# zkemail/zk-email-verify

Hardware: NVIDIA H100
Metric: EmailVerifier proofs/sec (witness+prove) (higher is better)
Workload: dtype u256 (BN254 Fr/Fq integers, 8x32-bit limbs)

## Files before the change

### zk-email-verify_b200/csrc/engine.cu

```cuda
#include "ff.cuh"
namespace zke { namespace dev { unsigned long long g_kernel_launches = 0; } }
#include "witness.cu"
#include "matvec.cu"
#include "ntt.cu"
#include "msm.cuh"
#include "fixed_base.cuh"
namespace zke { namespace dev {
ZKE_DEFINE_CONSTANT_UPLOAD(upload_constants_engine)
cudaError_t upload_constants_msm_g1(const FieldConsts*, const FieldConsts*);
cudaError_t upload_constants_msm_g2(const FieldConsts*, const FieldConsts*);
cudaError_t upload_constants_fixed_base(const FieldConsts*, const FieldConsts*);
cudaError_t upload_constants_verify(const FieldConsts*, const FieldConsts*);
} }

#include "../../include/zkemail_b200.h"
#include "cuda_host.hpp"
#include "engine.hpp"
#include "witness_program.hpp"
#include "binfile.hpp"
#include "ec_host.hpp"
#include "setup_host.hpp"
#include <algorithm>
#include <cstdio>
#include <cstring>
#include <atomic>
#include <memory>
#include <mutex>
#include <thread>
#include <unordered_map>

using namespace zke;

void zke::select_device(int device) {
    int n = 0;
    if (cudaGetDeviceCount(&n) != cudaSuccess || n == 0) throw std::runtime_error("no CUDA device available (this library has no CPU fallback)");
    if (device < 0 || device >= n) throw std::runtime_error("bad device index");
    CUDA_OK(cudaSetDevice(device));
    dev::FieldConsts fr, fq;
    fill_consts(fr, fr_params());
    fill_consts(fq, fq_params());
    CUDA_OK(dev::upload_constants_engine(&fr, &fq));
    CUDA_OK(dev::upload_constants_msm_g1(&fr, &fq));
    CUDA_OK(dev::upload_constants_msm_g2(&fr, &fq));
    CUDA_OK(dev::upload_constants_fixed_base(&fr, &fq));
    CUDA_OK(dev::upload_constants_verify(&fr, &fq));
    CUDA_OK(dev::configure_witness_kernel());
}

namespace {

template <class F>
std::vector<AffineH<F>> window_table(const AffineH<F>& gen) {
    std::vector<AffineH<F>> t(32 * 256, AffineH<F>::inf());
    JacobianH<F> base = JacobianH<F>::from_affine(gen);
    for (int w = 0; w < 32; ++w) {
        JacobianH<F> acc = JacobianH<F>::inf();
        for (int d = 1; d < 256; ++d) {
            acc = acc.add(base);
            t[w * 256 + d] = acc.to_affine();
        }
        for (int k = 0; k < 8; ++k) base = base.dbl();
    }
    return t;
}

std::vector<U256> to_standard(const std::vector<Fr>& v) {
    std::vector<U256> out(v.size());
    const unsigned T = std::max(1u, std::min(16u, std::thread::hardware_concurrency()));
    std::vector<std::thread> th;
    for (unsigned t = 0; t < T; ++t)
        th.emplace_back([&, t]() { for (size_t i = v.size() * t / T; i < v.size() * (t + 1) / T; ++i) out[i] = v[i].to_u256(); });
    for (auto& x : th) x.join();
    return out;
}

}

struct zke_zkey {
    uint32_t n_vars = 0, n_public = 0, log_n = 0;
    int device = 0;
    bool toy = false;
    bool delta_one = false;
    G1AffineH alpha1, beta1, delta1;
    G2AffineH beta2, gamma2, delta2;
    std::vector<G1AffineH> ic;
    DevBuf A, B1, B2, C, H;
    int h_levels = 1;
    dev::MsmConfig cfg_h;
    bool has_coefs = false;
    std::vector<uint32_t> a_ptr, a_var, a_coef, b_ptr, b_var, b_coef;
    std::vector<U256> coefs;
};

struct zke_ctx {
    const zke_circuit* circuit = nullptr;
    const zke_zkey* zkey = nullptr;
    int device = 0;
    uint32_t max_batch = 0;
    uint32_t n_vars = 0, n_public = 0, n_inputs = 0;
    cudaStream_t stream = nullptr;
    DevBuf ops, iter_hdr, lc_terms, aux, coop, coef_r, small_inv;
    std::vector<uint32_t> coef_word;
    std::vector<uint32_t> iter_info;
    DevBuf a_ptr, a_terms, b_ptr, b_terms, c_ptr, c_terms;
    dev::DevProgram prog;
    dev::DevR1cs r1cs;
    DevBuf tw_fwd, tw_inv, coset_scale;
    dev::NttTables ntt;
    size_t stride = 0;
    DevBuf inputs, check_flag;
    uint32_t inputs_resident = 0;
    struct Slot {
        bool allocated = false, busy = false;
        DevBuf w_all, inputs, results, first_bad;
        uint8_t* results_host = nullptr;
        uint8_t* publics_host = nullptr;
        std::vector<cudaEvent_t> done;
        cudaEvent_t witness_done = nullptr;
        uint32_t loaded = 0;
        uint32_t batch = 0;
        std::vector<uint8_t> rs;
    };
    Slot slots[2];
    uint64_t n_submitted = 0, n_collected = 0;
    int shard_rank = -1, shard_world = 0, shard_log_g = 0, shard_stage = 0;
    struct Lane { cudaStream_t st = nullptr, heavy = nullptr; cudaEvent_t ev[6] = {}; DevBuf va, vb, vc, vd, msm_ws; };
    Lane lanes[ZKE_MAX_LANES];
    int n_lanes = 1, lanes_alloc = 0;
    int finish_threads = 4;
    dev::MsmConfig cfg_w, cfg_h;
    bool split_streams = true;
    std::vector<uint32_t> bad_host;
    bool profile = false;
    std::vector<cudaEvent_t> ev_pool;
    size_t ev_used = 0;
    struct Span { int stage; size_t e0, e1; };
    std::vector<Span> spans;
    double stage_ms[ZKE_N_STAGES] = {0};
    uint64_t stage_count[ZKE_N_STAGES] = {0};
    cudaEvent_t ev(size_t* idx) {
        if (ev_used == ev_pool.size()) { cudaEvent_t e; cudaEventCreate(&e); ev_pool.push_back(e); }
        *idx = ev_used;
        return ev_pool[ev_used++];
    }
    size_t mark(cudaStream_t st) { size_t i; cudaEventRecord(ev(&i), st); return i; }
    size_t mark() { return mark(stream); }
    void collect() {
        for (auto& s : spans) {
            float ms = 0;
            if (cudaEventElapsedTime(&ms, ev_pool[s.e0], ev_pool[s.e1]) == cudaSuccess) { stage_ms[s.stage] += ms; stage_count[s.stage]++; }
        }
        spans.clear();
        ev_used = 0;
    }
};

static const uint32_t SETUP_SLAB = 1u << 20;
static void h_table_config(zke_zkey* zk, size_t N) {
    const char* e = getenv("ZKE_H_PRECOMP");
    const bool precomp = !(e && atoi(e) == 0);
    zk->cfg_h = dev::msm_config_full((uint32_t)N, precomp);
    zk->h_levels = precomp ? dev::msm_windows(zk->cfg_h) : 1;
}
static void build_h_levels(zke_zkey* zk, size_t N, uint8_t* scratch, cudaStream_t st) {
    for (int lvl = 1; lvl < zk->h_levels; ++lvl) {
        const uint8_t* prev = zk->H.p + (size_t)(lvl - 1) * N * sizeof(dev::G1Affine);
        uint8_t* cur = zk->H.p + (size_t)lvl * N * sizeof(dev::G1Affine);
        for (size_t off = 0; off < N; off += SETUP_SLAB) {
            uint32_t cnt = (uint32_t)std::min<size_t>(SETUP_SLAB, N - off);
            dev::scale_pow2_batch<dev::Fq>(prev + sizeof(dev::G1Affine) * off, cnt, zk->cfg_h.c, scratch, cur + sizeof(dev::G1Affine) * off, st);
        }
    }
    CHECK_LAUNCH();
    CUDA_OK(cudaStreamSynchronize(st));
}

static zke_zkey* do_setup(const zke_circuit* zc, uint64_t seed, int device) {
    select_device(device);
    const Circuit& c = zc->c;
    SetupScalars S = compute_setup_scalars(c, seed);
    std::unique_ptr<zke_zkey> zk(new zke_zkey());
    zk->n_vars = c.n_vars; zk->n_public = c.n_public(); zk->log_n = S.log_n; zk->device = device;
    zk->toy = true;
    const size_t N = (size_t)1 << S.log_n;
    const uint32_t m = c.n_vars, l = c.n_public();

    G1JacH g1 = G1JacH::from_affine(g1_generator());
    G2JacH g2 = G2JacH::from_affine(g2_generator());
    zk->alpha1 = g1.mul(S.alpha.to_u256()).to_affine();
    zk->beta1 = g1.mul(S.beta.to_u256()).to_affine();
    zk->delta1 = g1.mul(S.delta.to_u256()).to_affine();
    zk->beta2 = g2.mul(S.beta.to_u256()).to_affine();
    zk->gamma2 = g2.mul(S.gamma.to_u256()).to_affine();
    zk->delta2 = g2.mul(S.delta.to_u256()).to_affine();

    DevBuf t1, t2, scal, scratch;
    t1.upload(window_table<Fq>(g1_generator()));
    t2.upload(window_table<Fq2>(g2_generator()));
    const uint32_t SLAB = SETUP_SLAB;
    scratch.alloc((size_t)SLAB * sizeof(dev::G2XYZZ));
    cudaStream_t st = nullptr;

    auto run_g1 = [&](const std::vector<Fr>& s, DevBuf& out) {
        std::vector<U256> std_s = to_standard(s);
        scal.upload(std_s);
        out.alloc(s.size() * sizeof(dev::G1Affine));
        for (size_t off = 0; off < s.size(); off += SLAB) {
            uint32_t cnt = (uint32_t)std::min<size_t>(SLAB, s.size() - off);
            dev::fixed_base_batch<dev::Fq>(t1.p, scal.p + 32 * off, cnt, scratch.p, out.p + sizeof(dev::G1Affine) * off, st);
        }
        CHECK_LAUNCH();
        CUDA_OK(cudaStreamSynchronize(st));
    };
    run_g1(S.a, zk->A);
    run_g1(S.b, zk->B1);
    run_g1(S.kc, zk->C);
    {
        h_table_config(zk.get(), N);
        std::vector<U256> std_s = to_standard(S.h);
        scal.upload(std_s);
        zk->H.alloc((size_t)zk->h_levels * N * sizeof(dev::G1Affine));
        for (size_t off = 0; off < N; off += SLAB) {
            uint32_t cnt = (uint32_t)std::min<size_t>(SLAB, N - off);
            dev::fixed_base_batch<dev::Fq>(t1.p, scal.p + 32 * off, cnt, scratch.p, zk->H.p + sizeof(dev::G1Affine) * off, st);
        }
        build_h_levels(zk.get(), N, scratch.p, st);
    }
    {
        std::vector<U256> std_s = to_standard(S.b);
        scal.upload(std_s);
        zk->B2.alloc((size_t)m * sizeof(dev::G2Affine));
        for (size_t off = 0; off < m; off += SLAB) {
            uint32_t cnt = (uint32_t)std::min<size_t>(SLAB, m - off);
            dev::fixed_base_batch<dev::Fq2>(t2.p, scal.p + 32 * off, cnt, scratch.p, zk->B2.p + sizeof(dev::G2Affine) * off, st);
        }
        CHECK_LAUNCH();
        CUDA_OK(cudaStreamSynchronize(st));
    }
    zk->ic.resize(l + 1);
    CUDA_OK(cudaMemcpy(zk->ic.data(), zk->C.p, sizeof(G1AffineH) * (l + 1), cudaMemcpyDeviceToHost));
    CUDA_OK(cudaMemset(zk->C.p, 0, sizeof(G1AffineH) * (l + 1)));
    return zk.release();
}

namespace {
void split_container(const uint8_t* b, size_t len, SecView sec[11]) {
    if (!b || len < 12 || memcmp(b, "zkey", 4) != 0) throw std::runtime_error("not a .zkey file (bad magic)");
    if (rd32(b + 4) != 1) throw std::runtime_error("unsupported .zkey version");
    for (const BinSection& s : binfile_sections(b, len, ".zkey"))
        if (s.type >= 1 && s.type <= 10) sec[s.type] = s.view;
}

template <class Launch>
int64_t first_flagged(uint32_t* flag, Launch launch) {
    CUDA_OK(cudaMemset(flag, 0xff, 4));
    launch(flag);
    ZKE_COUNT_LAUNCH(1);
    CHECK_LAUNCH();
    uint32_t first = 0;
    CUDA_OK(cudaMemcpy(&first, flag, 4, cudaMemcpyDeviceToHost));
    return first == 0xffffffffu ? -1 : (int64_t)first;
}

template <class F>
__global__ void validate_points_kernel(const uint8_t* __restrict__ pts, uint32_t n, F b, uint32_t* bad) {
    const uint32_t i = blockIdx.x * blockDim.x + threadIdx.x;
    if (i >= n) return;
    const dev::Affine<F> p = dev::Affine<F>::load(pts + sizeof(dev::Affine<F>) * (size_t)i);
    if (p.is_inf()) return;
    if (!dev::below_modulus(p.x) || !dev::below_modulus(p.y) || !(p.y.sqr() == p.x.sqr() * p.x + b)) atomicMin(bad, i);
}

template <class F, class HostF>
int64_t first_invalid_point(const uint8_t* pts, size_t n, const HostF& b_host, uint32_t* flag) {
    if (!n) return -1;
    F b;
    static_assert(sizeof(F) == sizeof(HostF), "host / device field images differ");
    memcpy(&b, &b_host, sizeof(F));
    return first_flagged(flag, [&](uint32_t* f) { validate_points_kernel<F><<<(unsigned)((n + 127) / 128), 128>>>(pts, (uint32_t)n, b, f); });
}

Fq2 g2_twist_b() { return Fq2{Fq::from_u64(3), Fq::zero()} * Fq2{Fq::from_u64(9), Fq::one()}.inv(); }

struct U256HashE {
    size_t operator()(const U256& x) const { return (size_t)(x.v[0] * 0x9E3779B97F4A7C15ull ^ x.v[1] * 31 ^ x.v[2] * 131 ^ x.v[3]); }
};
}

static zke_zkey* do_zkey_load(const SecView sec[11], int device) {
    select_device(device);
    for (int s = 1; s <= 9; ++s) if (!sec[s].p) throw std::runtime_error(".zkey section " + std::to_string(s) + " is missing");
    if (sec[1].n < 4 || rd32(sec[1].p) != 1) throw std::runtime_error("not a Groth16 .zkey (protocol id)");
    const uint8_t* h = sec[2].p;
    const size_t HDR = 4 + 32 + 4 + 32 + 12 + 64 + 64 + 128 + 128 + 64 + 128;
    if (sec[2].n < HDR) throw std::runtime_error(".zkey header section too short");
    if (rd32(h) != 32 || memcmp(h + 4, fq_params().p.v, 32) != 0) throw std::runtime_error(".zkey is not over the BN254 base field");
    if (rd32(h + 36) != 32 || memcmp(h + 40, fr_params().p.v, 32) != 0) throw std::runtime_error(".zkey is not over the BN254 scalar field");
    std::unique_ptr<zke_zkey> zk(new zke_zkey());
    zk->device = device;
    zk->n_vars = rd32(h + 72); zk->n_public = rd32(h + 76);
    const uint32_t domain = rd32(h + 80);
    if (domain == 0 || (domain & (domain - 1)) || domain > (1u << 28)) throw std::runtime_error(".zkey domain size is not a power of two <= 2^28");
    zk->log_n = 0;
    while ((1u << zk->log_n) < domain) zk->log_n++;
    const uint32_t m = zk->n_vars, l = zk->n_public;
    if (m == 0 || l + 1 > m) throw std::runtime_error(".zkey header: nPublic + 1 > nVars");
    const size_t N = domain;
    auto need = [&](int s, size_t bytes) {
        if (sec[s].n != bytes) throw std::runtime_error(".zkey section " + std::to_string(s) + " has " + std::to_string(sec[s].n) + " bytes, expected " + std::to_string(bytes));
    };
    need(3, (size_t)(l + 1) * 64); need(5, (size_t)m * 64); need(6, (size_t)m * 64); need(7, (size_t)m * 128);
    need(8, (size_t)(m - l - 1) * 64); need(9, N * 64);

    const uint8_t* q = h + 84;
    memcpy(&zk->alpha1, q, 64); memcpy(&zk->beta1, q + 64, 64); memcpy(&zk->beta2, q + 128, 128);
    memcpy(&zk->gamma2, q + 256, 128); memcpy(&zk->delta1, q + 384, 64); memcpy(&zk->delta2, q + 448, 128);
    auto fq_ok = [](const Fq& x) { return u256_cmp(x.m, fq_params().p) < 0; };
    auto g1_ok = [&](const G1AffineH& p) { return fq_ok(p.x) && fq_ok(p.y) && g1_on_curve(p); };
    auto g2_ok = [&](const G2AffineH& p) { return fq_ok(p.x.c0) && fq_ok(p.x.c1) && fq_ok(p.y.c0) && fq_ok(p.y.c1) && g2_on_curve(p); };
    if (!g1_ok(zk->alpha1) || !g1_ok(zk->beta1) || !g1_ok(zk->delta1) || !g2_ok(zk->beta2) || !g2_ok(zk->gamma2) || !g2_ok(zk->delta2))
        throw std::runtime_error(".zkey header: a key point is not on its curve");
    zk->ic.resize(l + 1);
    memcpy(zk->ic.data(), sec[3].p, (size_t)(l + 1) * 64);
    for (auto& p : zk->ic) if (!g1_ok(p)) throw std::runtime_error(".zkey section 3: an IC point is not on the curve");

    {
        if (sec[4].n < 4) throw std::runtime_error(".zkey section 4 too short");
        const uint32_t n_rec = rd32(sec[4].p);
        if (sec[4].n != 4 + (size_t)n_rec * 44) throw std::runtime_error(".zkey section 4: size does not match its record count");
        const uint8_t* rec = sec[4].p + 4;
        zk->a_ptr.assign(N + 1, 0); zk->b_ptr.assign(N + 1, 0);
        for (uint32_t k = 0; k < n_rec; ++k) {
            const uint8_t* r = rec + 44 * (size_t)k;
            const uint32_t mat = rd32(r), row = rd32(r + 4), sig = rd32(r + 8);
            if (mat > 1 || row >= N || sig >= m) throw std::runtime_error(".zkey section 4: record " + std::to_string(k) + " out of range");
            (mat == 0 ? zk->a_ptr : zk->b_ptr)[row + 1]++;
        }
        for (size_t i = 0; i < N; ++i) { zk->a_ptr[i + 1] += zk->a_ptr[i]; zk->b_ptr[i + 1] += zk->b_ptr[i]; }
        zk->a_var.resize(zk->a_ptr[N]); zk->a_coef.resize(zk->a_ptr[N]);
        zk->b_var.resize(zk->b_ptr[N]); zk->b_coef.resize(zk->b_ptr[N]);
        std::vector<uint32_t> ca(zk->a_ptr.begin(), zk->a_ptr.end() - 1), cb(zk->b_ptr.begin(), zk->b_ptr.end() - 1);
        const Fr r_elem = Fr::from_u256(fr_params().r);
        const Fr rinv2 = (r_elem * r_elem).inv();
        std::unordered_map<U256, uint32_t, U256HashE> index;
        for (uint32_t k = 0; k < n_rec; ++k) {
            const uint8_t* r = rec + 44 * (size_t)k;
            const uint32_t mat = rd32(r), row = rd32(r + 4), sig = rd32(r + 8);
            U256 raw;
            memcpy(raw.v, r + 12, 32);
            auto it = index.find(raw);
            if (it == index.end()) {
                if (u256_cmp(raw, fr_params().p) >= 0) throw std::runtime_error(".zkey section 4: coefficient not reduced mod r");
                it = index.emplace(raw, (uint32_t)zk->coefs.size()).first;
                zk->coefs.push_back((Fr::from_u256(raw) * rinv2).to_u256());
            }
            if (mat == 0) { const uint32_t pos = ca[row]++; zk->a_var[pos] = sig; zk->a_coef[pos] = it->second; }
            else { const uint32_t pos = cb[row]++; zk->b_var[pos] = sig; zk->b_coef[pos] = it->second; }
        }
        if (zk->coefs.size() >= (1u << 24)) throw std::runtime_error(".zkey has more than 2^24 distinct coefficients");
        zk->has_coefs = true;
    }

    DevBuf flag, scratch;
    flag.alloc(4);
    const Fq b1 = Fq::from_u64(3);
    const Fq2 b2 = g2_twist_b();
    auto up = [&](DevBuf& dst, const uint8_t* src, size_t bytes, size_t skip) {
        dst.alloc(skip + bytes);
        if (skip) CUDA_OK(cudaMemset(dst.p, 0, skip));
        if (bytes) CUDA_OK(cudaMemcpy(dst.p + skip, src, bytes, cudaMemcpyHostToDevice));
    };
    auto refuse = [](int64_t bad, const char* what) {
        if (bad >= 0) throw std::runtime_error(std::string(".zkey section ") + what + ": point " + std::to_string(bad) + " is not on the curve");
    };
    uint32_t* fl = (uint32_t*)flag.p;
    up(zk->A, sec[5].p, sec[5].n, 0);   refuse(first_invalid_point<dev::Fq>(zk->A.p, m, b1, fl), "5 (A)");
    up(zk->B1, sec[6].p, sec[6].n, 0);  refuse(first_invalid_point<dev::Fq>(zk->B1.p, m, b1, fl), "6 (B1)");
    up(zk->B2, sec[7].p, sec[7].n, 0);  refuse(first_invalid_point<dev::Fq2>(zk->B2.p, m, b2, fl), "7 (B2)");
    up(zk->C, sec[8].p, sec[8].n, (size_t)(l + 1) * 64);
    refuse(first_invalid_point<dev::Fq>(zk->C.p, m, b1, fl), "8 (C)");
    h_table_config(zk.get(), N);
    zk->H.alloc((size_t)zk->h_levels * N * sizeof(dev::G1Affine));
    CUDA_OK(cudaMemcpy(zk->H.p, sec[9].p, N * 64, cudaMemcpyHostToDevice));
    refuse(first_invalid_point<dev::Fq>(zk->H.p, N, b1, fl), "9 (H)");
    scratch.alloc((size_t)SETUP_SLAB * sizeof(dev::G1XYZZ));
    build_h_levels(zk.get(), N, scratch.p, nullptr);
    return zk.release();
}

static int64_t do_zkey_write(const zke_zkey* zk, const zke_circuit* zc, uint8_t* out, size_t cap) {
    const uint32_t m = zk->n_vars, l = zk->n_public;
    const size_t N = (size_t)1 << zk->log_n;
    const Circuit* c = zc ? &zc->c : nullptr;
    if (!zk->has_coefs) {
        if (!c) throw std::runtime_error("a key made by zke_setup needs its circuit to write the coefficient section");
        if (c->n_vars != m || c->n_public() != l || c->domain_log2() != zk->log_n) throw std::runtime_error("zkey does not belong to this circuit");
    }
    size_t n_rec;
    if (zk->has_coefs) n_rec = zk->a_var.size() + zk->b_var.size();
    else n_rec = c->a_var.size() + c->b_var.size() + l + 1;
    const size_t HDR = 4 + 32 + 4 + 32 + 12 + 64 + 64 + 128 + 128 + 64 + 128;
    const size_t sizes[11] = {0, 4, HDR, (size_t)(l + 1) * 64, 4 + n_rec * 44, (size_t)m * 64, (size_t)m * 64, (size_t)m * 128,
                              (size_t)(m - l - 1) * 64, N * 64, 68};
    size_t total = 12;
    for (int s = 1; s <= 10; ++s) total += 12 + sizes[s];
    if (!out) return (int64_t)total;
    if (cap < total) return -2;
    CUDA_OK(cudaSetDevice(zk->device));
    BinWriter w{out};
    w.header("zkey", 1, 10);
    w.section(1, sizes[1]); w.u32(1);
    w.section(2, sizes[2]);
    w.u32(32); w.bytes(fq_params().p.v, 32); w.u32(32); w.bytes(fr_params().p.v, 32); w.u32(m); w.u32(l); w.u32((uint32_t)N);
    w.bytes(&zk->alpha1, 64); w.bytes(&zk->beta1, 64); w.bytes(&zk->beta2, 128); w.bytes(&zk->gamma2, 128); w.bytes(&zk->delta1, 64); w.bytes(&zk->delta2, 128);
    w.section(3, sizes[3]); w.bytes(zk->ic.data(), (size_t)(l + 1) * 64);
    w.section(4, sizes[4]); w.u32((uint32_t)n_rec);
    {
        const std::vector<U256>& coefs = zk->has_coefs ? zk->coefs : c->coefs;
        const Fr r_elem = Fr::from_u256(fr_params().r);
        const Fr r2 = r_elem * r_elem;
        std::vector<U256> stored(coefs.size());
        for (size_t i = 0; i < coefs.size(); ++i) stored[i] = (Fr::from_u256(coefs[i]) * r2).to_u256();
        auto rows = [&](uint32_t mat, const std::vector<uint32_t>& ptr, const std::vector<uint32_t>& var, const std::vector<uint32_t>& coef, size_t n_rows) {
            for (size_t row = 0; row < n_rows; ++row)
                for (uint32_t k = ptr[row]; k < ptr[row + 1]; ++k) { w.u32(mat); w.u32((uint32_t)row); w.u32(var[k]); w.bytes(stored[coef[k]].v, 32); }
        };
        if (zk->has_coefs) {
            rows(0, zk->a_ptr, zk->a_var, zk->a_coef, N);
            rows(1, zk->b_ptr, zk->b_var, zk->b_coef, N);
        } else {
            rows(0, c->a_ptr, c->a_var, c->a_coef, c->n_constraints);
            rows(1, c->b_ptr, c->b_var, c->b_coef, c->n_constraints);
            const U256 one_r2 = r2.to_u256();
            for (uint32_t j = 0; j <= l; ++j) { w.u32(0); w.u32(c->n_constraints + j); w.u32(j); w.bytes(one_r2.v, 32); }
        }
    }
    auto dev_sec = [&](int s, const DevBuf& b, size_t skip) {
        w.section(s, sizes[s]);
        if (sizes[s]) CUDA_OK(cudaMemcpy(w.p, b.p + skip, sizes[s], cudaMemcpyDeviceToHost));
        w.p += sizes[s];
    };
    dev_sec(5, zk->A, 0); dev_sec(6, zk->B1, 0); dev_sec(7, zk->B2, 0); dev_sec(8, zk->C, (size_t)(l + 1) * 64); dev_sec(9, zk->H, 0);
    w.section(10, sizes[10]); memset(w.p, 0, 68); w.p += 68;
    return (int64_t)(w.p - out);
}

static void alloc_slot(zke_ctx* x, zke_ctx::Slot& S) {
    if (S.allocated) return;
    S.w_all.alloc(x->stride * 32 * x->max_batch);
    S.inputs.alloc((size_t)std::max(1u, x->n_inputs) * 32 * x->max_batch);
    S.first_bad.alloc(4 * (size_t)x->max_batch);
    if (x->zkey) {
        S.results.alloc((size_t)x->max_batch * ZKE_RESULT_STRIDE);
        CUDA_OK(cudaHostAlloc((void**)&S.results_host, (size_t)x->max_batch * ZKE_RESULT_STRIDE, cudaHostAllocDefault));
        CUDA_OK(cudaHostAlloc((void**)&S.publics_host, (size_t)x->max_batch * std::max(1u, x->n_public) * 32, cudaHostAllocDefault));
        S.done.resize(x->max_batch);
        for (auto& e : S.done) CUDA_OK(cudaEventCreateWithFlags(&e, cudaEventDisableTiming));
        CUDA_OK(cudaEventCreateWithFlags(&S.witness_done, cudaEventDisableTiming));
    }
    S.allocated = true;
}

static void check_key_matrices(const Circuit& c, const zke_zkey& zk) {
    const size_t N = (size_t)1 << zk.log_n;
    const uint32_t nc = c.n_constraints, l = c.n_public();
    typedef std::vector<std::pair<uint32_t, Fr>> Form;
    auto canonical = [](Form& f) {
        std::sort(f.begin(), f.end(), [](const std::pair<uint32_t, Fr>& a, const std::pair<uint32_t, Fr>& b) { return a.first < b.first; });
        size_t o = 0;
        for (size_t i = 0; i < f.size();) {
            std::pair<uint32_t, Fr> t = f[i++];
            while (i < f.size() && f[i].first == t.first) t.second = t.second + f[i++].second;
            if (!t.second.is_zero()) f[o++] = t;
        }
        f.resize(o);
    };
    Form x, y;
    auto compare = [&](const char* name, const std::vector<uint32_t>& kp, const std::vector<uint32_t>& kv, const std::vector<uint32_t>& kc,
                       const std::vector<uint32_t>& cp, const std::vector<uint32_t>& cv, const std::vector<uint32_t>& cc, bool extra) {
        for (size_t row = 0; row < N; ++row) {
            const uint32_t kb = kp[row], ke = kp[row + 1];
            if (row < nc) {
                const uint32_t b = cp[row], e = cp[row + 1];
                bool same = e - b == ke - kb;
                for (uint32_t k = 0; same && k < e - b; ++k) same = cv[b + k] == kv[kb + k] && c.coefs[cc[b + k]] == zk.coefs[kc[kb + k]];
                if (same) continue;
            }
            x.clear(); y.clear();
            for (uint32_t k = kb; k < ke; ++k) x.emplace_back(kv[k], Fr::from_u256(zk.coefs[kc[k]]));
            if (row < nc) {
                for (uint32_t k = cp[row]; k < cp[row + 1]; ++k) y.emplace_back(cv[k], Fr::from_u256(c.coefs[cc[k]]));
            } else if (extra && row <= (size_t)nc + l) {
                y.emplace_back((uint32_t)(row - nc), Fr::one());
            }
            canonical(x); canonical(y);
            bool same = x.size() == y.size();
            for (size_t i = 0; same && i < x.size(); ++i) same = x[i].first == y[i].first && x[i].second == y[i].second;
            if (!same) throw std::runtime_error(std::string("zkey does not belong to this circuit: ") + name + " row " + std::to_string(row) + " differs");
        }
    };
    compare("A", zk.a_ptr, zk.a_var, zk.a_coef, c.a_ptr, c.a_var, c.a_coef, true);
    compare("B", zk.b_ptr, zk.b_var, zk.b_coef, c.b_ptr, c.b_var, c.b_coef, false);
}

static void upload_program(zke_ctx* x, const Circuit& c) {
    const uint32_t max_batch = x->max_batch;
    LowerOptions opt;
    if (const char* e = getenv("ZKE_NATIVE_SHA")) opt.native_sha = atoi(e) != 0;
    if (const char* e = getenv("ZKE_NATIVE_REGEX")) opt.native_regex = atoi(e) != 0;
    if (const char* e = getenv("ZKE_COOP_FPMUL")) opt.coop_fpmul = atoi(e) != 0;
    const uint32_t sms = (uint32_t)dev::sm_count();
    opt.cluster = max_batch <= 8 ? 8 : (max_batch <= 32 ? 4 : (2 * max_batch <= sms ? 2 : 1));
    if (const char* e = getenv("ZKE_WITNESS_CLUSTER")) { const int v = atoi(e); if (v == 1 || v == 2 || v == 4 || v == 8) opt.cluster = (uint32_t)v; }
    WitnessStream S = lower_witness_program(c, x->coef_word, opt);
    x->ops.upload(S.ops);
    x->iter_hdr.upload(S.iter_hdr);
    x->lc_terms.upload(S.terms);
    x->aux.upload(S.aux);
    x->coop.upload(S.coop);
    x->iter_info = std::move(S.iter_info);
    const uint32_t NSMALL = 4096;
    std::vector<Fr> inv(NSMALL);
    for (uint32_t i = 0; i < NSMALL; ++i) inv[i] = Fr::from_u64(i);
    batch_inverse(inv.data(), NSMALL);
    std::vector<U256> inv_std(NSMALL);
    for (uint32_t i = 0; i < NSMALL; ++i) inv_std[i] = inv[i].to_u256();
    x->small_inv.upload(inv_std);
    dev::DevProgram& P = x->prog;
    P.ops = (const uint4*)x->ops.p; P.iter_hdr = (const uint4*)x->iter_hdr.p; P.coop = (const uint32_t*)x->coop.p;
    P.terms = (const uint2*)x->lc_terms.p; P.aux = (const uint32_t*)x->aux.p; P.coef_r = x->coef_r.p;
    P.small_inv = x->small_inv.p; P.n_small_inv = NSMALL;
    P.trace = nullptr;
    P.cluster = S.cluster;
    P.n_iters = S.n_iters; P.n_ops = (uint32_t)c.ops.size(); P.n_vars = c.n_vars; P.n_temps = c.n_temps;
    P.n_outputs = c.n_outputs; P.n_inputs = c.n_inputs();
}

static void upload_r1cs(zke_ctx* x, const Circuit* cp, const zke_zkey* zk) {
    auto up_terms = [&](const std::vector<uint32_t>& var, const std::vector<uint32_t>& coef, DevBuf& dst) {
        std::vector<uint32_t> t(2 * var.size() + 2);
        for (size_t i = 0; i < var.size(); ++i) { t[2 * i] = var[i]; t[2 * i + 1] = x->coef_word[coef[i]]; }
        dst.upload(t);
    };
    dev::DevR1cs& R = x->r1cs;
    if (cp) {
        const Circuit& c = *cp;
        x->a_ptr.upload(c.a_ptr); x->b_ptr.upload(c.b_ptr); x->c_ptr.upload(c.c_ptr);
        up_terms(c.a_var, c.a_coef, x->a_terms); up_terms(c.b_var, c.b_coef, x->b_terms); up_terms(c.c_var, c.c_coef, x->c_terms);
        R.c_ptr = (const uint32_t*)x->c_ptr.p; R.c_terms = (const uint2*)x->c_terms.p;
        R.n_constraints = c.n_constraints; R.n_public = c.n_public();
    } else {
        x->a_ptr.upload(zk->a_ptr); x->b_ptr.upload(zk->b_ptr);
        up_terms(zk->a_var, zk->a_coef, x->a_terms); up_terms(zk->b_var, zk->b_coef, x->b_terms);
        R.c_ptr = nullptr; R.c_terms = nullptr;
        R.n_constraints = 1u << zk->log_n; R.n_public = 0;
    }
    R.a_ptr = (const uint32_t*)x->a_ptr.p; R.b_ptr = (const uint32_t*)x->b_ptr.p;
    R.a_terms = (const uint2*)x->a_terms.p; R.b_terms = (const uint2*)x->b_terms.p;
    R.coef_r = x->coef_r.p; R.n_vars = x->n_vars;
}

namespace {
struct ShoupPair { U256 w, wq; };
U256 mul_lo256(const U256& a, const U256& b) {
    uint64_t t[4] = {0, 0, 0, 0};
    for (int i = 0; i < 4; ++i) {
        u128 c = 0;
        for (int j = 0; i + j < 4; ++j) {
            c += (u128)a.v[j] * b.v[i] + t[i + j];
            t[i + j] = (uint64_t)c;
            c >>= 64;
        }
    }
    return U256{{t[0], t[1], t[2], t[3]}};
}
const U256& fr_neg_inv256() {
    static const U256 v = [] {
        const U256& p = fr_params().p;
        U256 y = {{(uint64_t)0 - fr_params().inv, 0, 0, 0}};
        for (int it = 0; it < 2; ++it) {
            U256 t = mul_lo256(p, y), two = {{2, 0, 0, 0}}, d;
            u256_sub(d, two, t);
            y = mul_lo256(y, d);
        }
        U256 zero = {{0, 0, 0, 0}}, n;
        u256_sub(n, zero, y);
        return n;
    }();
    return v;
}
ShoupPair shoup_pair(const Fr& w) { return ShoupPair{w.to_u256(), mul_lo256(w.m, fr_neg_inv256())}; }
}

static void build_ntt_tables(zke_ctx* x, unsigned log_n) {
    const size_t N = (size_t)1 << log_n;
    const Fr omega = fr_root_of_unity(log_n), omega_inv = omega.inv();
    const Fr g = fr_root_of_unity(log_n + 1);
    const Fr n_inv = Fr::from_u64(N).inv();
    bool shoup = false;
    if (const char* e = getenv("ZKE_NTT_SHOUP")) shoup = atoi(e) != 0;
    const size_t esz = shoup ? 64 : 32;
    std::vector<uint8_t> fw(esz * std::max<size_t>(1, N / 2)), iv(esz * std::max<size_t>(1, N / 2)), cs(esz * N);
    auto put = [&](std::vector<uint8_t>& tab, size_t i, const Fr& w) {
        if (shoup) { const ShoupPair sp = shoup_pair(w); memcpy(&tab[64 * i], sp.w.v, 32); memcpy(&tab[64 * i + 32], sp.wq.v, 32); }
        else memcpy(&tab[32 * i], w.m.v, 32);
    };
    const unsigned T = std::max(1u, std::min(16u, std::thread::hardware_concurrency()));
    std::vector<std::thread> th;
    for (unsigned t = 0; t < T; ++t) {
        th.emplace_back([&, t]() {
            size_t beg = (N / 2) * t / T, end = (N / 2) * (t + 1) / T;
            if (beg < end) {
                U256 e = {{(uint64_t)beg, 0, 0, 0}};
                Fr a = omega.pow(e), b = omega_inv.pow(e);
                for (size_t i = beg; i < end; ++i) { put(fw, i, a); put(iv, i, b); a = a * omega; b = b * omega_inv; }
            }
            beg = N * t / T; end = N * (t + 1) / T;
            if (beg < end) {
                U256 e = {{(uint64_t)beg, 0, 0, 0}};
                Fr a = g.pow(e) * n_inv;
                for (size_t j = beg; j < end; ++j) {
                    size_t p = 0;
                    for (unsigned bit = 0; bit < log_n; ++bit) if (j & ((size_t)1 << bit)) p |= (size_t)1 << (log_n - 1 - bit);
                    put(cs, p, a);
                    a = a * g;
                }
            }
        });
    }
    for (auto& t : th) t.join();
    if (N == 1) { put(fw, 0, Fr::one()); put(iv, 0, Fr::one()); }
    x->tw_fwd.upload(fw); x->tw_inv.upload(iv); x->coset_scale.upload(cs);
    x->ntt.tw_fwd = x->tw_fwd.p; x->ntt.tw_inv = x->tw_inv.p; x->ntt.log_n = (int)log_n; x->ntt.shoup = shoup;
}

static void open_lanes(zke_ctx* x, size_t N, int prio_least, int prio_greatest) {
    const uint32_t max_batch = x->max_batch;
    x->cfg_w = dev::msm_config_witness();
    x->cfg_h = x->zkey->cfg_h;
    size_t ws = std::max(dev::MsmPlan<dev::Fq>::workspace_bytes(x->n_vars, x->cfg_w),
                         dev::MsmPlan<dev::Fq>::workspace_bytes((uint32_t)N, x->cfg_h));
    ws = std::max(ws, dev::MsmPlan<dev::Fq2>::workspace_bytes(x->n_vars, x->cfg_w));
    int want = 8;
    if (const char* e = getenv("ZKE_LANES")) want = atoi(e);
    if (const char* e = getenv("ZKE_SPLIT_STREAMS")) x->split_streams = atoi(e) != 0;
    if (const char* e = getenv("ZKE_FINISH_THREADS")) x->finish_threads = std::max(1, std::min(32, atoi(e)));
    want = std::max(1, std::min(ZKE_MAX_LANES, std::min<int>(want, (int)max_batch)));
    {
        size_t free_b = 0, total_b = 0;
        CUDA_OK(cudaMemGetInfo(&free_b, &total_b));
        const size_t lane_bytes = 4 * N * 32 + ws;
        const size_t keep = x->stride * 32 * max_batch + ((size_t)1 << 30);
        const size_t fit = free_b > keep ? (free_b - keep) / lane_bytes : 0;
        want = std::max(1, std::min<int>(want, (int)std::min<size_t>(fit, ZKE_MAX_LANES)));
    }
    const int prio_light = prio_greatest < prio_least - 1 ? prio_greatest + 1 : prio_greatest;
    for (int i = 0; i < want; ++i) {
        zke_ctx::Lane& L = x->lanes[i];
        CUDA_OK(cudaStreamCreateWithPriority(&L.st, cudaStreamNonBlocking, prio_light));
        CUDA_OK(cudaStreamCreateWithPriority(&L.heavy, cudaStreamNonBlocking, prio_least));
        for (auto& e : L.ev) CUDA_OK(cudaEventCreateWithFlags(&e, cudaEventDisableTiming));
        L.va.alloc(N * 32); L.vb.alloc(N * 32); L.vc.alloc(N * 32); L.vd.alloc(N * 32);
        L.msm_ws.alloc(ws);
    }
    x->lanes_alloc = x->n_lanes = want;
}

static zke_ctx* do_open(const zke_circuit* zc, const zke_zkey* zk, int device, uint32_t max_batch) {
    select_device(device);
    const Circuit* cp = zc ? &zc->c : nullptr;
    if (!cp && !(zk && zk->has_coefs)) throw std::runtime_error("a context needs a circuit, or a proving key loaded from a .zkey");
    if (zk && cp && (zk->n_vars != cp->n_vars || zk->n_public != cp->n_public() || zk->log_n != cp->domain_log2()))
        throw std::runtime_error("zkey does not belong to this circuit");
    if (zk && zk->device != device) throw std::runtime_error("zkey lives on another device");
    if (max_batch == 0) throw std::runtime_error("max_batch must be positive");
    std::unique_ptr<zke_ctx> x(new zke_ctx());
    x->circuit = zc; x->zkey = zk; x->device = device; x->max_batch = max_batch;
    x->n_vars = cp ? cp->n_vars : zk->n_vars;
    x->n_public = cp ? cp->n_public() : zk->n_public;
    x->n_inputs = cp ? cp->n_inputs() : 0;
    int prio_least = 0, prio_greatest = 0;
    CUDA_OK(cudaDeviceGetStreamPriorityRange(&prio_least, &prio_greatest));
    CUDA_OK(cudaStreamCreateWithPriority(&x->stream, cudaStreamNonBlocking, prio_greatest));

    const std::vector<U256>& coefs = cp ? cp->coefs : zk->coefs;
    x->coef_word = coef_words(coefs);
    {
        std::vector<Fr> cr(std::max<size_t>(1, coefs.size()));
        for (size_t i = 0; i < coefs.size(); ++i) cr[i] = Fr::from_u256(coefs[i]);
        x->coef_r.upload(cr);
    }

    if (zk && cp && cp->r1cs_only && zk->has_coefs) check_key_matrices(*cp, *zk);

    if (cp && !cp->r1cs_only) upload_program(x.get(), *cp);
    upload_r1cs(x.get(), cp, zk);
    x->stride = (size_t)x->n_vars + (cp ? cp->n_temps : 0);
    x->inputs.alloc((size_t)std::max(1u, x->n_inputs) * 32 * max_batch);
    x->check_flag.alloc(8);
    x->bad_host.resize(max_batch);
    alloc_slot(x.get(), x->slots[0]);

    if (zk) {
        build_ntt_tables(x.get(), zk->log_n);
        open_lanes(x.get(), (size_t)1 << zk->log_n, prio_least, prio_greatest);
    }
    CUDA_OK(cudaDeviceSynchronize());
    return x.release();
}

static std::string assert_message(const zke_ctx* x, uint32_t email, uint32_t row) {
    std::string scope = "?";
    if (x->circuit) {
        const Circuit& c = x->circuit->c;
        if (row < c.scope_of_constraint.size()) scope = c.scopes[c.scope_of_constraint[row]];
    }
    return "Assert Failed: constraint " + std::to_string(row) + " in template " + scope + " @ email " + std::to_string(email);
}

static void require_idle(const zke_ctx* x) {
    if (x->n_submitted != x->n_collected) throw std::runtime_error("a submitted batch is still in flight: call zke_fullprove_collect first");
}

static void do_witness(zke_ctx* x, zke_ctx::Slot& S, const uint8_t* inputs, size_t batch) {
    if (!x->circuit) throw std::runtime_error("this context was opened from a .zkey alone: it has no witness program (use zke_load_witness / zke_wtns_prove)");
    const Circuit& c = x->circuit->c;
    if (c.r1cs_only) throw std::runtime_error(R1CS_NO_PROGRAM);
    if (batch == 0 || batch > x->max_batch) throw std::runtime_error("batch exceeds the context's max_batch");
    CUDA_OK(cudaSetDevice(x->device));
    const uint8_t* in_dev = x->inputs.p;
    if (inputs) {
        if (c.n_inputs()) CUDA_OK(cudaMemcpyAsync(S.inputs.p, inputs, (size_t)c.n_inputs() * 32 * batch, cudaMemcpyHostToDevice, x->stream));
        in_dev = S.inputs.p;
    } else if (x->inputs_resident < batch) {
        throw std::runtime_error("inputs == NULL but no (or too few) inputs are resident: call zke_upload_inputs first");
    }
    size_t p0 = 0;
    if (x->profile) p0 = x->mark();
    if (const char* tp = getenv("ZKE_WITNESS_TRACE")) {
        DevBuf tr;
        tr.alloc(8 * ((size_t)x->prog.n_iters + 1));
        dev::DevProgram P = x->prog;
        P.trace = (unsigned long long*)tr.p;
        dev::launch_witness(P, S.w_all.p, x->stride, in_dev, (uint32_t)batch, x->stream);
        CUDA_OK(cudaStreamSynchronize(x->stream));
        std::vector<unsigned long long> h(x->prog.n_iters);
        CUDA_OK(cudaMemcpy(h.data(), tr.p, 8 * h.size(), cudaMemcpyDeviceToHost));
        if (FILE* f = fopen(tp, "wb")) {
            fwrite(h.data(), 8, h.size(), f);
            fwrite(x->iter_info.data(), 4, x->iter_info.size(), f);
            fclose(f);
        }
    }
    dev::launch_witness(x->prog, S.w_all.p, x->stride, in_dev, (uint32_t)batch, x->stream);
    CHECK_LAUNCH();
    if (x->profile) x->spans.push_back({ZKE_STAGE_WITNESS, p0, x->mark()});
    S.loaded = (uint32_t)batch;
}

static int do_check(zke_ctx* x, zke_ctx::Slot& S, size_t batch, int32_t* status, std::string& msg) {
    CUDA_OK(cudaMemsetAsync(S.first_bad.p, 0xff, 4 * batch, x->stream));
    dev::launch_check_rows(x->r1cs, S.w_all.p, x->stride, (uint32_t)batch, (uint32_t*)S.first_bad.p, x->stream);
    CHECK_LAUNCH();
    CUDA_OK(cudaMemcpyAsync(x->bad_host.data(), S.first_bad.p, 4 * batch, cudaMemcpyDeviceToHost, x->stream));
    CUDA_OK(cudaStreamSynchronize(x->stream));
    if (x->profile) x->collect();
    int bad = 0;
    for (size_t e = 0; e < batch; ++e) {
        int32_t s = x->bad_host[e] == 0xffffffffu ? -1 : (int32_t)x->bad_host[e];
        if (status) status[e] = s;
        if (s >= 0) { if (!bad) msg = assert_message(x, (uint32_t)e, (uint32_t)s); ++bad; }
    }
    return bad;
}

static void write_fq(uint8_t* dst, const Fq& x) { U256 s = x.to_u256(); memcpy(dst, s.v, 32); }

template <class F>
static AffineH<F> finish_msm(const uint8_t* block, const dev::MsmConfig& cfg) {
    const XyzzH<F>* slots = reinterpret_cast<const XyzzH<F>*>(block);
    const int n_windows = cfg.precomputed ? 1 : (255 + cfg.c - 1) / cfg.c;
    XyzzH<F> acc = XyzzH<F>::inf();
    for (int j = n_windows - 1; j >= 0; --j) {
        if (!acc.is_inf()) for (int k = 0; k < cfg.c; ++k) acc.dbl();
        acc.add(slots[dev::MSM_ONES_SLOTS + j]);
    }
    if (cfg.classify) for (int i = 0; i < dev::MSM_ONES_SLOTS; ++i) acc.add(slots[i]);
    return acc.to_affine();
}

static void sync_lanes(zke_ctx* x) {
    cudaStreamSynchronize(x->stream);
    for (int i = 0; i < x->lanes_alloc; ++i) { cudaStreamSynchronize(x->lanes[i].st); cudaStreamSynchronize(x->lanes[i].heavy); }
}

static void enqueue_prove(zke_ctx* x, zke_ctx::Slot& S, size_t batch, const uint8_t* rs) {
    const zke_zkey* zk = x->zkey;
    if (!zk) throw std::runtime_error("context was opened without a proving key");
    if (batch == 0 || batch > S.loaded) throw std::runtime_error("no witness loaded for this batch (call zke_witness first)");
    if (rs) {
        for (size_t e = 0; e < 2 * batch; ++e) {
            U256 v;
            memcpy(v.v, rs + 32 * e, 32);
            if (u256_cmp(v, fr_params().p) >= 0) throw std::runtime_error("r / s not reduced mod the group order");
        }
        S.rs.assign(rs, rs + 64 * batch);
    } else {
        S.rs.clear();
    }
    CUDA_OK(cudaSetDevice(x->device));
    const uint32_t N = 1u << zk->log_n, m = x->n_vars, l = x->n_public;
    const bool prof = x->profile;
    const int n_lanes = prof ? 1 : x->n_lanes;
    if (const char* e = getenv("ZKE_SPLIT_STREAMS")) x->split_streams = atoi(e) != 0;
    if (l) CUDA_OK(cudaMemcpy2DAsync(S.publics_host, (size_t)l * 32, S.w_all.p + 32, x->stride * 32, (size_t)l * 32, batch, cudaMemcpyDeviceToHost, x->stream));
    CUDA_OK(cudaEventRecord(S.witness_done, x->stream));
    for (int i = 0; i < n_lanes; ++i) CUDA_OK(cudaStreamWaitEvent(x->lanes[i].st, S.witness_done, 0));
    for (size_t e = 0; e < batch; ++e) {
        zke_ctx::Lane& L = x->lanes[e % n_lanes];
        cudaStream_t st = L.st;
        const uint8_t* w = S.w_all.p + 32 * x->stride * e;
        uint8_t* res = S.results.p + (size_t)ZKE_RESULT_STRIDE * e;
        uint32_t* flag = (uint32_t*)(res + ZKE_RES_FLAG_OFF);
        size_t t0 = 0, t1 = 0;
        CUDA_OK(cudaMemsetAsync(flag, 0xff, 4, st));
        if (prof) t0 = x->mark(st);
        cudaStream_t hv = (prof || !x->split_streams) ? st : L.heavy;
        dev::launch_build_ab(x->r1cs, w, L.va.p, L.vb.p, L.vc.p, N, flag, st);
        if (prof) { t1 = x->mark(st); x->spans.push_back({ZKE_STAGE_MATVEC, t0, t1}); t0 = t1; }
        if (hv != st) { CUDA_OK(cudaEventRecord(L.ev[0], st)); CUDA_OK(cudaStreamWaitEvent(hv, L.ev[0], 0)); }
        dev::launch_intt_dif(L.va.p, x->ntt, x->coset_scale.p, hv);
        dev::launch_intt_dif(L.vb.p, x->ntt, x->coset_scale.p, hv);
        dev::launch_intt_dif(L.vc.p, x->ntt, x->coset_scale.p, hv);
        dev::launch_ntt_dit(L.va.p, x->ntt, hv);
        dev::launch_ntt_dit(L.vb.p, x->ntt, hv);
        dev::launch_ntt_dit(L.vc.p, x->ntt, hv);
        dev::launch_quotient(L.va.p, L.vb.p, L.vc.p, L.vd.p, N, hv);
        CHECK_LAUNCH();
        if (hv != st) CUDA_OK(cudaEventRecord(L.ev[1], hv));
        if (prof) { t1 = x->mark(st); x->spans.push_back({ZKE_STAGE_NTT, t0, t1}); t0 = t1; }
        uint8_t* ws_w = L.msm_ws.p;
        dev::MsmPlan<dev::Fq>::run(zk->A.p, w, m, x->cfg_w, ws_w, res + 0 * ZKE_RES_G1_BLOCK, st);
        if (prof) { t1 = x->mark(st); x->spans.push_back({ZKE_STAGE_MSM_A, t0, t1}); t0 = t1; }
        dev::MsmPlan<dev::Fq>::run(zk->B1.p, w, m, x->cfg_w, ws_w, res + 1 * ZKE_RES_G1_BLOCK, st);
        if (prof) { t1 = x->mark(st); x->spans.push_back({ZKE_STAGE_MSM_B1, t0, t1}); t0 = t1; }
        dev::MsmPlan<dev::Fq>::run(zk->C.p, w, m, x->cfg_w, ws_w, res + 2 * ZKE_RES_G1_BLOCK, st);
        if (prof) { t1 = x->mark(st); x->spans.push_back({ZKE_STAGE_MSM_C, t0, t1}); t0 = t1; }
        dev::MsmPlan<dev::Fq2>::run(zk->B2.p, w, m, x->cfg_w, ws_w, res + 4 * ZKE_RES_G1_BLOCK, st);
        CHECK_LAUNCH();
        if (prof) { t1 = x->mark(st); x->spans.push_back({ZKE_STAGE_MSM_B2, t0, t1}); t0 = t1; }
        if (hv != st) CUDA_OK(cudaStreamWaitEvent(st, L.ev[1], 0));
        {
            dev::MsmPlan<dev::Fq>::Heavy heavy{hv, L.ev[2], L.ev[3]};
            if (prof) {
                size_t i0, i1;
                cudaEvent_t evs[2];
                evs[0] = x->ev(&i0); evs[1] = x->ev(&i1);
                dev::MsmPlan<dev::Fq>::run(zk->H.p, L.vd.p, N, x->cfg_h, L.msm_ws.p, res + 3 * ZKE_RES_G1_BLOCK, st, evs, &heavy);
                x->spans.push_back({ZKE_STAGE_MSM_H_BUCKETS, i0, i1});
                t1 = x->mark(st); x->spans.push_back({ZKE_STAGE_MSM_H, t0, t1}); t0 = t1;
            } else {
                dev::MsmPlan<dev::Fq>::run(zk->H.p, L.vd.p, N, x->cfg_h, L.msm_ws.p, res + 3 * ZKE_RES_G1_BLOCK, st, nullptr, &heavy);
            }
        }
        CHECK_LAUNCH();
        CUDA_OK(cudaMemcpyAsync(S.results_host + (size_t)ZKE_RESULT_STRIDE * e, res, ZKE_RESULT_STRIDE, cudaMemcpyDeviceToHost, st));
        CUDA_OK(cudaEventRecord(S.done[e], st));
    }
    S.batch = (uint32_t)batch;
}

static int finish_prove(zke_ctx* x, zke_ctx::Slot& S, uint8_t* proofs_out, uint8_t* publics_out, int32_t* status, std::string& msg) {
    const zke_zkey* zk = x->zkey;
    const size_t batch = S.batch;
    const uint32_t l = x->n_public;
    const G1JacH alpha1 = G1JacH::from_affine(zk->alpha1), beta1 = G1JacH::from_affine(zk->beta1), delta1 = G1JacH::from_affine(zk->delta1);
    const G2JacH beta2 = G2JacH::from_affine(zk->beta2), delta2 = G2JacH::from_affine(zk->delta2);
    std::vector<int32_t> st_local(batch, -1);
    std::string first_error;
    std::mutex err_mutex;
    auto one = [&](size_t e) {
        CUDA_OK(cudaEventSynchronize(S.done[e]));
        const uint8_t* res = S.results_host + (size_t)ZKE_RESULT_STRIDE * e;
        uint32_t flag;
        memcpy(&flag, res + ZKE_RES_FLAG_OFF, 4);
        const int32_t s = flag == 0xffffffffu ? -1 : (int32_t)flag;
        st_local[e] = s;
        uint8_t* out = proofs_out + 256 * e;
        if (s >= 0) { memset(out, 0, 256); return; }
        U256 r, sc;
        if (!S.rs.empty()) { memcpy(r.v, S.rs.data() + 64 * e, 32); memcpy(sc.v, S.rs.data() + 64 * e + 32, 32); }
        else { random_scalar(r); random_scalar(sc); }
        G1AffineH ma = finish_msm<Fq>(res + 0 * ZKE_RES_G1_BLOCK, x->cfg_w);
        G1AffineH mb1 = finish_msm<Fq>(res + 1 * ZKE_RES_G1_BLOCK, x->cfg_w);
        G1AffineH mc = finish_msm<Fq>(res + 2 * ZKE_RES_G1_BLOCK, x->cfg_w);
        G1AffineH mh = finish_msm<Fq>(res + 3 * ZKE_RES_G1_BLOCK, x->cfg_h);
        G2AffineH mb2 = finish_msm<Fq2>(res + 4 * ZKE_RES_G1_BLOCK, x->cfg_w);
        G1JacH pa = alpha1.add(G1JacH::from_affine(ma)).add(delta1.mul(r));
        G2JacH pb2 = beta2.add(G2JacH::from_affine(mb2)).add(delta2.mul(sc));
        G1JacH pb1 = beta1.add(G1JacH::from_affine(mb1)).add(delta1.mul(sc));
        U256 rs_prod = (Fr::from_u256(r) * Fr::from_u256(sc)).to_u256();
        G1JacH pc = G1JacH::from_affine(mc).add(G1JacH::from_affine(mh)).add(pa.mul(sc)).add(pb1.mul(r)).add(delta1.mul(rs_prod).neg());
        G1AffineH A = pa.to_affine(), C = pc.to_affine();
        G2AffineH B = pb2.to_affine();
        write_fq(out + 0, A.x); write_fq(out + 32, A.y);
        write_fq(out + 64, B.x.c0); write_fq(out + 96, B.x.c1); write_fq(out + 128, B.y.c0); write_fq(out + 160, B.y.c1);
        write_fq(out + 192, C.x); write_fq(out + 224, C.y);
    };
    const int T = (int)std::max<size_t>(1, std::min<size_t>((size_t)x->finish_threads, batch));
    std::atomic<size_t> next{0};
    auto worker = [&]() {
        try {
            cudaSetDevice(x->device);
            for (;;) {
                const size_t e = next.fetch_add(1);
                if (e >= batch) break;
                one(e);
            }
        } catch (const std::exception& ex) {
            std::lock_guard<std::mutex> lock(err_mutex);
            if (first_error.empty()) first_error = ex.what();
        }
    };
    if (T == 1) worker();
    else {
        std::vector<std::thread> th;
        for (int t = 0; t < T; ++t) th.emplace_back(worker);
        for (auto& t : th) t.join();
    }
    if (x->profile) { sync_lanes(x); x->collect(); }
    if (!first_error.empty()) { sync_lanes(x); throw std::runtime_error(first_error); }
    int bad = 0;
    for (size_t e = 0; e < batch; ++e) {
        if (status) status[e] = st_local[e];
        if (st_local[e] >= 0) { if (!bad) msg = assert_message(x, (uint32_t)e, (uint32_t)st_local[e]); ++bad; }
    }
    if (publics_out && l) memcpy(publics_out, S.publics_host, (size_t)l * 32 * batch);
    return bad;
}

static int do_prove(zke_ctx* x, zke_ctx::Slot& S, size_t batch, const uint8_t* rs, uint8_t* proofs_out, uint8_t* publics_out, int32_t* status, std::string& msg) {
    try {
        enqueue_prove(x, S, batch, rs);
    } catch (...) {
        sync_lanes(x);
        throw;
    }
    return finish_prove(x, S, proofs_out, publics_out, status, msg);
}

static const uint8_t* parse_wtns(const uint8_t* b, size_t len, uint32_t expect_vars) {
    if (!b || len < 12 || memcmp(b, "wtns", 4) != 0) throw std::runtime_error("not a .wtns file (bad magic)");
    std::vector<BinSection> secs;
    try { secs = binfile_sections(b, len, ".wtns"); }
    catch (const std::runtime_error&) { throw std::runtime_error("truncated .wtns"); }
    const uint8_t *s1 = nullptr, *s2 = nullptr;
    size_t n1 = 0, n2 = 0;
    for (const BinSection& s : secs) {
        if (s.type == 1) { s1 = s.view.p; n1 = s.view.n; }
        if (s.type == 2) { s2 = s.view.p; n2 = s.view.n; }
    }
    if (!s1 || !s2 || n1 < 40) throw std::runtime_error(".wtns sections missing");
    if (rd32(s1) != 32 || memcmp(s1 + 4, fr_params().p.v, 32) != 0) throw std::runtime_error(".wtns is not over the BN254 scalar field");
    const uint32_t n = rd32(s1 + 36);
    if (n != expect_vars) throw std::runtime_error(".wtns has " + std::to_string(n) + " values, the key expects " + std::to_string(expect_vars));
    if (n2 != (size_t)n * 32) throw std::runtime_error(".wtns data section has the wrong size");
    return s2;
}

static void load_witness(zke_ctx* x, zke_ctx::Slot& S, const uint8_t* wtns, size_t batch) {
    if (batch == 0 || batch > x->max_batch) throw std::runtime_error("batch exceeds the context's max_batch");
    CUDA_OK(cudaSetDevice(x->device));
    const size_t m = x->n_vars;
    CUDA_OK(cudaMemcpy2DAsync(S.w_all.p, x->stride * 32, wtns, m * 32, m * 32, batch, cudaMemcpyHostToDevice, x->stream));
    CUDA_OK(cudaMemsetAsync(x->check_flag.p, 0, 8, x->stream));
    dev::launch_check_witness(S.w_all.p, x->stride, (uint32_t)m, (uint32_t)batch, (uint32_t*)x->check_flag.p, x->stream);
    CHECK_LAUNCH();
    uint32_t flags[2] = {0, 0};
    CUDA_OK(cudaMemcpyAsync(flags, x->check_flag.p, 8, cudaMemcpyDeviceToHost, x->stream));
    CUDA_OK(cudaStreamSynchronize(x->stream));
    S.loaded = 0;
    if (flags[0]) throw std::runtime_error("witness value not reduced mod r");
    if (flags[1]) throw std::runtime_error("witness[0] must be 1");
    S.loaded = (uint32_t)batch;
}

static void shard_geometry(const zke_ctx* x, int& log_m, int& log_cols, uint32_t& col0) {
    log_m = (int)x->zkey->log_n - x->shard_log_g;
    log_cols = log_m - x->shard_log_g;
    col0 = (uint32_t)x->shard_rank << log_cols;
}

static void shard_begin(zke_ctx* x, int rank, int world) {
    const zke_zkey* zk = x->zkey;
    if (!zk) throw std::runtime_error("context was opened without a proving key");
    require_idle(x);
    int log_g = 0;
    while ((1 << log_g) < world) ++log_g;
    if (world < 2 || world > 8 || (1 << log_g) != world) throw std::runtime_error("sharded proving supports 2, 4 or 8 GPUs");
    if (rank < 0 || rank >= world) throw std::runtime_error("bad shard rank");
    if ((int)zk->log_n < 2 * log_g + 10) throw std::runtime_error("domain too small to shard (use batch parallelism)");
    zke_ctx::Slot& S = x->slots[0];
    if (S.loaded < 1) throw std::runtime_error("no witness loaded (call zke_witness / zke_load_witness on every rank first)");
    CUDA_OK(cudaSetDevice(x->device));
    x->shard_rank = rank; x->shard_world = world; x->shard_log_g = log_g;
    int log_m, log_cols; uint32_t col0;
    shard_geometry(x, log_m, log_cols, col0);
    zke_ctx::Lane& L = x->lanes[0];
    cudaStream_t st = L.st;
    CUDA_OK(cudaStreamSynchronize(x->stream));
    uint32_t* flag = (uint32_t*)(S.results.p + ZKE_RES_FLAG_OFF);
    CUDA_OK(cudaMemsetAsync(flag, 0xff, 4, st));
    dev::RowMap map;
    map.log_cols = log_cols; map.log_m = log_m; map.col0 = col0;
    const uint32_t n_rows = (uint32_t)world << log_cols;
    dev::launch_build_ab(x->r1cs, S.w_all.p, L.va.p, L.vb.p, L.vc.p, n_rows, flag, st, &map);
    const uint32_t n_cols = 1u << log_cols;
    dev::launch_intt_cross(L.va.p, x->ntt, log_g, col0, n_cols, st);
    dev::launch_intt_cross(L.vb.p, x->ntt, log_g, col0, n_cols, st);
    dev::launch_intt_cross(L.vc.p, x->ntt, log_g, col0, n_cols, st);
    CHECK_LAUNCH();
    CUDA_OK(cudaStreamSynchronize(st));
    x->shard_stage = 1;
}

static void shard_mid(zke_ctx* x) {
    if (x->shard_stage != 1) throw std::runtime_error("zke_shard_mid out of order");
    CUDA_OK(cudaSetDevice(x->device));
    int log_m, log_cols; uint32_t col0;
    shard_geometry(x, log_m, log_cols, col0);
    zke_ctx::Lane& L = x->lanes[0];
    cudaStream_t st = L.st;
    const size_t block_off = ((size_t)x->shard_rank << log_m);
    for (uint8_t* v : {L.va.p, L.vb.p, L.vc.p}) {
        dev::launch_intt_dif_block(v + 32 * block_off, x->ntt, log_m, x->coset_scale.p + (x->ntt.shoup ? 64 : 32) * block_off, st);
        dev::launch_ntt_dit_block(v + 32 * block_off, x->ntt, log_m, st);
    }
    CHECK_LAUNCH();
    CUDA_OK(cudaStreamSynchronize(st));
    x->shard_stage = 2;
}

static void put_g1(uint8_t* dst, const G1AffineH& p) { write_fq(dst, p.x); write_fq(dst + 32, p.y); }

static void shard_end(zke_ctx* x, uint8_t* partial_out, uint8_t* publics_out) {
    if (x->shard_stage != 2) throw std::runtime_error("zke_shard_end out of order");
    const zke_zkey* zk = x->zkey;
    CUDA_OK(cudaSetDevice(x->device));
    int log_m, log_cols; uint32_t col0;
    shard_geometry(x, log_m, log_cols, col0);
    zke_ctx::Slot& S = x->slots[0];
    zke_ctx::Lane& L = x->lanes[0];
    cudaStream_t st = L.st;
    const uint32_t N = 1u << zk->log_n, m = x->n_vars, l = x->n_public;
    const int G = x->shard_world, log_g = x->shard_log_g;
    const uint32_t n_cols = 1u << log_cols;
    dev::launch_ntt_cross(L.va.p, x->ntt, log_g, col0, n_cols, st);
    dev::launch_ntt_cross(L.vb.p, x->ntt, log_g, col0, n_cols, st);
    dev::launch_ntt_cross(L.vc.p, x->ntt, log_g, col0, n_cols, st);
    CUDA_OK(cudaMemsetAsync(L.vd.p, 0, (size_t)N * 32, st));
    dev::launch_quotient_cols(L.va.p, L.vb.p, L.vc.p, L.vd.p, (int)zk->log_n, log_g, col0, (uint32_t)log_cols, st);
    CHECK_LAUNCH();
    const uint32_t lo = (uint32_t)((uint64_t)m * x->shard_rank / G), hi = (uint32_t)((uint64_t)m * (x->shard_rank + 1) / G);
    const uint8_t* w = S.w_all.p;
    uint8_t* res = S.results.p;
    dev::MsmPlan<dev::Fq>::run(zk->A.p + 64ull * lo, w + 32ull * lo, hi - lo, x->cfg_w, L.msm_ws.p, res + 0 * ZKE_RES_G1_BLOCK, st);
    dev::MsmPlan<dev::Fq>::run(zk->B1.p + 64ull * lo, w + 32ull * lo, hi - lo, x->cfg_w, L.msm_ws.p, res + 1 * ZKE_RES_G1_BLOCK, st);
    dev::MsmPlan<dev::Fq>::run(zk->C.p + 64ull * lo, w + 32ull * lo, hi - lo, x->cfg_w, L.msm_ws.p, res + 2 * ZKE_RES_G1_BLOCK, st);
    dev::MsmPlan<dev::Fq2>::run(zk->B2.p + 128ull * lo, w + 32ull * lo, hi - lo, x->cfg_w, L.msm_ws.p, res + 4 * ZKE_RES_G1_BLOCK, st);
    dev::MsmPlan<dev::Fq>::run(zk->H.p, L.vd.p, N, x->cfg_h, L.msm_ws.p, res + 3 * ZKE_RES_G1_BLOCK, st);
    CHECK_LAUNCH();
    CUDA_OK(cudaMemcpyAsync(S.results_host, res, ZKE_RESULT_STRIDE, cudaMemcpyDeviceToHost, st));
    if (l) CUDA_OK(cudaMemcpyAsync(S.publics_host, S.w_all.p + 32, (size_t)l * 32, cudaMemcpyDeviceToHost, st));
    CUDA_OK(cudaStreamSynchronize(st));
    const uint8_t* rh = S.results_host;
    put_g1(partial_out + 0, finish_msm<Fq>(rh + 0 * ZKE_RES_G1_BLOCK, x->cfg_w));
    put_g1(partial_out + 64, finish_msm<Fq>(rh + 1 * ZKE_RES_G1_BLOCK, x->cfg_w));
    put_g1(partial_out + 128, finish_msm<Fq>(rh + 2 * ZKE_RES_G1_BLOCK, x->cfg_w));
    put_g1(partial_out + 192, finish_msm<Fq>(rh + 3 * ZKE_RES_G1_BLOCK, x->cfg_h));
    const G2AffineH b2 = finish_msm<Fq2>(rh + 4 * ZKE_RES_G1_BLOCK, x->cfg_w);
    write_fq(partial_out + 256, b2.x.c0); write_fq(partial_out + 288, b2.x.c1); write_fq(partial_out + 320, b2.y.c0); write_fq(partial_out + 352, b2.y.c1);
    memcpy(partial_out + 384, rh + ZKE_RES_FLAG_OFF, 4);
    if (publics_out && l) memcpy(publics_out, S.publics_host, (size_t)l * 32);
    x->shard_stage = 0;
}

static Fq fq_from_le(const uint8_t* b) {
    U256 v;
    memcpy(v.v, b, 32);
    if (u256_cmp(v, fq_params().p) >= 0) throw std::runtime_error("partial point coordinate not reduced");
    return Fq::from_u256(v);
}

struct ShardKeyPoints { G1AffineH alpha1, beta1, delta1; G2AffineH beta2, delta2; };
static int shard_combine(const ShardKeyPoints* zk, const uint8_t* partials, int world, const uint8_t* rs, uint8_t* out, int32_t* status) {
    G1JacH sa = G1JacH::inf(), sb1 = G1JacH::inf(), sc = G1JacH::inf(), sh = G1JacH::inf();
    G2JacH sb2 = G2JacH::inf();
    uint32_t first_bad = 0xffffffffu;
    for (int r = 0; r < world; ++r) {
        const uint8_t* p = partials + (size_t)ZKE_SHARD_PARTIAL_BYTES * r;
        auto g1 = [&](const uint8_t* q) { return G1AffineH{fq_from_le(q), fq_from_le(q + 32)}; };
        const G1AffineH a = g1(p), b1 = g1(p + 64), c = g1(p + 128), h = g1(p + 192);
        const G2AffineH b2{Fq2{fq_from_le(p + 256), fq_from_le(p + 288)}, Fq2{fq_from_le(p + 320), fq_from_le(p + 352)}};
        if (!g1_on_curve(a) || !g1_on_curve(b1) || !g1_on_curve(c) || !g1_on_curve(h) || !g2_on_curve(b2)) throw std::runtime_error("partial point not on the curve");
        sa = sa.add_affine(a); sb1 = sb1.add_affine(b1); sc = sc.add_affine(c); sh = sh.add_affine(h); sb2 = sb2.add_affine(b2);
        uint32_t f;
        memcpy(&f, p + 384, 4);
        first_bad = std::min(first_bad, f);
    }
    if (status) *status = first_bad == 0xffffffffu ? -1 : (int32_t)first_bad;
    if (first_bad != 0xffffffffu) { memset(out, 0, 256); return 1; }
    U256 r, s;
    if (rs) { memcpy(r.v, rs, 32); memcpy(s.v, rs + 32, 32); }
    else { random_scalar(r); random_scalar(s); }
    if (u256_cmp(r, fr_params().p) >= 0 || u256_cmp(s, fr_params().p) >= 0) throw std::runtime_error("r / s not reduced mod the group order");
    const G1JacH alpha1 = G1JacH::from_affine(zk->alpha1), beta1 = G1JacH::from_affine(zk->beta1), delta1 = G1JacH::from_affine(zk->delta1);
    const G2JacH beta2 = G2JacH::from_affine(zk->beta2), delta2 = G2JacH::from_affine(zk->delta2);
    G1JacH pa = alpha1.add(sa).add(delta1.mul(r));
    G2JacH pb2 = beta2.add(sb2).add(delta2.mul(s));
    G1JacH pb1 = beta1.add(sb1).add(delta1.mul(s));
    U256 rs_prod = (Fr::from_u256(r) * Fr::from_u256(s)).to_u256();
    G1JacH pc = sc.add(sh).add(pa.mul(s)).add(pb1.mul(r)).add(delta1.mul(rs_prod).neg());
    G1AffineH A = pa.to_affine(), C = pc.to_affine();
    G2AffineH B = pb2.to_affine();
    write_fq(out + 0, A.x); write_fq(out + 32, A.y);
    write_fq(out + 64, B.x.c0); write_fq(out + 96, B.x.c1); write_fq(out + 128, B.y.c0); write_fq(out + 160, B.y.c1);
    write_fq(out + 192, C.x); write_fq(out + 224, C.y);
    return 0;
}

extern "C" {

int zke_device_count(void) {
    int n = 0;
    if (cudaGetDeviceCount(&n) != cudaSuccess) return 0;
    return n;
}

zke_zkey* zke_setup(const zke_circuit* c, uint64_t seed, int device, char* err, size_t errcap) {
    try { if (!c) throw std::runtime_error("null circuit"); return do_setup(c, seed, device); }
    catch (const std::exception& e) { set_err(err, errcap, e.what()); return nullptr; }
}
zke_zkey* zke_zkey_load(const void* zkey_bytes, size_t len, int device, char* err, size_t errcap) {
    try {
        SecView sec[11];
        split_container((const uint8_t*)zkey_bytes, len, sec);
        return do_zkey_load(sec, device);
    } catch (const std::exception& e) { set_err(err, errcap, e.what()); return nullptr; }
}
zke_zkey* zke_zkey_load_chunks(const void* const* chunks, const size_t* lens, size_t n_chunks, int device, char* err, size_t errcap) {
    try {
        if (!chunks || !lens || n_chunks < 9) throw std::runtime_error("expected the chunk files b..j (sections 1-9; k is optional)");
        SecView sec[11];
        for (size_t i = 0; i < n_chunks && i < 10; ++i) sec[i + 1] = SecView{(const uint8_t*)chunks[i], lens[i]};
        return do_zkey_load(sec, device);
    } catch (const std::exception& e) { set_err(err, errcap, e.what()); return nullptr; }
}
int64_t zke_zkey_write(const zke_zkey* z, const zke_circuit* c, uint8_t* out, size_t cap) {
    try { if (!z) return -1; return do_zkey_write(z, c, out, cap); }
    catch (const std::exception&) { return -3; }
}
int zke_zkey_is_toy(const zke_zkey* z) { return z ? (z->toy ? 1 : 0) : -1; }
void zke_zkey_free(zke_zkey* z) { if (z) { cudaSetDevice(z->device); delete z; } }

int zke_zkey_info(const zke_zkey* z, uint32_t* n_vars, uint32_t* n_public, uint32_t* domain_log2) {
    if (!z) return -1;
    if (n_vars) *n_vars = z->n_vars;
    if (n_public) *n_public = z->n_public;
    if (domain_log2) *domain_log2 = z->log_n;
    return 0;
}

int64_t zke_zkey_section(const zke_zkey* z, int section, uint8_t* out, size_t cap) {
    if (!z) return -1;
    try {
        CUDA_OK(cudaSetDevice(z->device));
        const size_t N = (size_t)1 << z->log_n;
        auto g1_host = [&](const G1AffineH* pts, size_t n) -> int64_t {
            if (!out) return (int64_t)n;
            if (cap < n * 64) return -2;
            for (size_t i = 0; i < n; ++i) { write_fq(out + 64 * i, pts[i].x); write_fq(out + 64 * i + 32, pts[i].y); }
            return (int64_t)n;
        };
        auto g1_dev = [&](const DevBuf& b, size_t n) -> int64_t {
            if (!out) return (int64_t)n;
            std::vector<G1AffineH> h(n);
            CUDA_OK(cudaMemcpy(h.data(), b.p, n * sizeof(G1AffineH), cudaMemcpyDeviceToHost));
            return g1_host(h.data(), n);
        };
        auto g2_host = [&](const G2AffineH* pts, size_t n) -> int64_t {
            if (!out) return (int64_t)n;
            if (cap < n * 128) return -2;
            for (size_t i = 0; i < n; ++i) {
                write_fq(out + 128 * i, pts[i].x.c0); write_fq(out + 128 * i + 32, pts[i].x.c1);
                write_fq(out + 128 * i + 64, pts[i].y.c0); write_fq(out + 128 * i + 96, pts[i].y.c1);
            }
            return (int64_t)n;
        };
        switch (section) {
            case ZKE_SEC_ALPHA1: return g1_host(&z->alpha1, 1);
            case ZKE_SEC_BETA1: return g1_host(&z->beta1, 1);
            case ZKE_SEC_DELTA1: return g1_host(&z->delta1, 1);
            case ZKE_SEC_BETA2: return g2_host(&z->beta2, 1);
            case ZKE_SEC_GAMMA2: return g2_host(&z->gamma2, 1);
            case ZKE_SEC_DELTA2: return g2_host(&z->delta2, 1);
            case ZKE_SEC_IC: return g1_host(z->ic.data(), z->ic.size());
            case ZKE_SEC_A: return g1_dev(z->A, z->n_vars);
            case ZKE_SEC_B1: return g1_dev(z->B1, z->n_vars);
            case ZKE_SEC_C: return g1_dev(z->C, z->n_vars);
            case ZKE_SEC_H: return g1_dev(z->H, N);
            case ZKE_SEC_B2: {
                if (!out) return z->n_vars;
                std::vector<G2AffineH> h(z->n_vars);
                CUDA_OK(cudaMemcpy(h.data(), z->B2.p, h.size() * sizeof(G2AffineH), cudaMemcpyDeviceToHost));
                return g2_host(h.data(), h.size());
            }
            default: return -1;
        }
    } catch (const std::exception&) { return -3; }
}

zke_ctx* zke_ctx_open(const zke_circuit* c, const zke_zkey* zkey, int device, uint32_t max_batch, char* err, size_t errcap) {
    try { return do_open(c, zkey, device, max_batch); }
    catch (const std::exception& e) { set_err(err, errcap, e.what()); return nullptr; }
}
void zke_ctx_close(zke_ctx* x) {
    if (!x) return;
    cudaSetDevice(x->device);
    sync_lanes(x);
    for (auto e : x->ev_pool) cudaEventDestroy(e);
    for (auto& S : x->slots) {
        for (auto e : S.done) cudaEventDestroy(e);
        if (S.witness_done) cudaEventDestroy(S.witness_done);
        if (S.results_host) cudaFreeHost(S.results_host);
        if (S.publics_host) cudaFreeHost(S.publics_host);
    }
    for (int i = 0; i < x->lanes_alloc; ++i) {
        if (x->lanes[i].st) cudaStreamDestroy(x->lanes[i].st);
        if (x->lanes[i].heavy) cudaStreamDestroy(x->lanes[i].heavy);
        for (auto e : x->lanes[i].ev) if (e) cudaEventDestroy(e);
    }
    if (x->stream) cudaStreamDestroy(x->stream);
    delete x;
}

int zke_upload_inputs(zke_ctx* x, const uint8_t* inputs, size_t batch, char* err, size_t errcap) {
    try {
        if (!x || !inputs) throw std::runtime_error("null argument");
        if (x->circuit && x->circuit->c.r1cs_only) throw std::runtime_error(R1CS_NO_PROGRAM);
        if (batch == 0 || batch > x->max_batch) throw std::runtime_error("batch exceeds the context's max_batch");
        require_idle(x);
        CUDA_OK(cudaSetDevice(x->device));
        const size_t n = x->n_inputs;
        if (n) CUDA_OK(cudaMemcpy(x->inputs.p, inputs, n * 32 * batch, cudaMemcpyHostToDevice));
        x->inputs_resident = (uint32_t)batch;
        return 0;
    } catch (const std::exception& e) { set_err(err, errcap, e.what()); return -1; }
}

int zke_ctx_set_lanes(zke_ctx* x, int n) {
    if (!x || n < 1) return -1;
    x->n_lanes = n > x->lanes_alloc ? x->lanes_alloc : n;
    return x->n_lanes;
}
int zke_ctx_profile(zke_ctx* x, int enable) {
    if (!x) return -1;
    x->profile = enable != 0;
    for (int i = 0; i < ZKE_N_STAGES; ++i) { x->stage_ms[i] = 0; x->stage_count[i] = 0; }
    return 0;
}
int zke_ctx_profile_get(const zke_ctx* x, double* ms_out, uint64_t* count_out) {
    if (!x) return -1;
    for (int i = 0; i < ZKE_N_STAGES; ++i) { if (ms_out) ms_out[i] = x->stage_ms[i]; if (count_out) count_out[i] = x->stage_count[i]; }
    return ZKE_N_STAGES;
}
void* zke_ctx_stream(const zke_ctx* x) { return x ? (void*)x->stream : nullptr; }
uint64_t zke_kernel_launches(void) { return dev::g_kernel_launches; }

int zke_witness(zke_ctx* x, const uint8_t* inputs, size_t batch, uint8_t* wtns_out, int32_t* status, char* err, size_t errcap) {
    try {
        if (!x) throw std::runtime_error("null context");
        require_idle(x);
        zke_ctx::Slot& S = x->slots[0];
        do_witness(x, S, inputs, batch);
        std::string msg;
        int bad = do_check(x, S, batch, status, msg);
        if (wtns_out) {
            const size_t m = x->n_vars;
            CUDA_OK(cudaMemcpy2D(wtns_out, m * 32, S.w_all.p, x->stride * 32, m * 32, batch, cudaMemcpyDeviceToHost));
        }
        if (bad) { set_err(err, errcap, msg); return bad; }
        return 0;
    } catch (const std::exception& e) { set_err(err, errcap, e.what()); return -1; }
}

int zke_load_witness(zke_ctx* x, const uint8_t* wtns, size_t batch, char* err, size_t errcap) {
    try {
        if (!x || !wtns) throw std::runtime_error("null argument");
        require_idle(x);
        load_witness(x, x->slots[0], wtns, batch);
        return 0;
    } catch (const std::exception& e) { set_err(err, errcap, e.what()); return -1; }
}

int zke_check_witness(zke_ctx* x, size_t batch, int32_t* status, char* err, size_t errcap) {
    try {
        if (!x) throw std::runtime_error("null context");
        if (!x->circuit) throw std::runtime_error("this context was opened from a .zkey alone: it has no C matrix to check witnesses against (open it with the circuit)");
        require_idle(x);
        zke_ctx::Slot& S = x->slots[0];
        if (batch == 0 || batch > S.loaded) throw std::runtime_error("no witness loaded for this batch (call zke_load_witness first)");
        CUDA_OK(cudaSetDevice(x->device));
        std::string msg;
        int bad = do_check(x, S, batch, status, msg);
        if (bad) { set_err(err, errcap, msg); return bad; }
        return 0;
    } catch (const std::exception& e) { set_err(err, errcap, e.what()); return -1; }
}

int zke_prove(zke_ctx* x, size_t batch, const uint8_t* rs, uint8_t* proofs_out, uint8_t* publics_out, int32_t* status, char* err, size_t errcap) {
    try {
        if (!x || !proofs_out) throw std::runtime_error("null argument");
        require_idle(x);
        std::string msg;
        int bad = do_prove(x, x->slots[0], batch, rs, proofs_out, publics_out, status, msg);
        if (bad) { set_err(err, errcap, msg); return bad; }
        return 0;
    } catch (const std::exception& e) { set_err(err, errcap, e.what()); return -1; }
}

int zke_wtns_prove(zke_ctx* x, const void* wtns_bytes, size_t len, const uint8_t* rs, uint8_t* proof_out, uint8_t* publics_out,
                   char* err, size_t errcap) {
    try {
        if (!x || !proof_out) throw std::runtime_error("null argument");
        require_idle(x);
        const uint8_t* data = parse_wtns((const uint8_t*)wtns_bytes, len, x->n_vars);
        load_witness(x, x->slots[0], data, 1);
        std::string msg;
        int32_t status = -1;
        int bad = do_prove(x, x->slots[0], 1, rs, proof_out, publics_out, &status, msg);
        if (bad) { set_err(err, errcap, msg); return bad; }
        return 0;
    } catch (const std::exception& e) { set_err(err, errcap, e.what()); return -1; }
}

int zke_fullprove_submit(zke_ctx* x, const uint8_t* inputs, size_t batch, const uint8_t* rs, char* err, size_t errcap) {
    try {
        if (!x) throw std::runtime_error("null context");
        if (x->profile) throw std::runtime_error("stage profiling needs the synchronous entry points");
        if (x->n_submitted - x->n_collected >= 2) throw std::runtime_error("two batches are already in flight: collect one first");
        CUDA_OK(cudaSetDevice(x->device));
        zke_ctx::Slot& S = x->slots[x->n_submitted & 1];
        alloc_slot(x, S);
        try {
            do_witness(x, S, inputs, batch);
            enqueue_prove(x, S, batch, rs);
        } catch (...) { sync_lanes(x); throw; }
        S.busy = true;
        x->n_submitted++;
        return 0;
    } catch (const std::exception& e) { set_err(err, errcap, e.what()); return -1; }
}

int zke_fullprove_collect(zke_ctx* x, uint8_t* proofs_out, uint8_t* publics_out, int32_t* status, char* err, size_t errcap) {
    try {
        if (!x || !proofs_out) throw std::runtime_error("null argument");
        if (x->n_submitted == x->n_collected) throw std::runtime_error("nothing was submitted");
        zke_ctx::Slot& S = x->slots[x->n_collected & 1];
        x->n_collected++;
        S.busy = false;
        std::string msg;
        int bad = finish_prove(x, S, proofs_out, publics_out, status, msg);
        if (bad) { set_err(err, errcap, msg); return bad; }
        return 0;
    } catch (const std::exception& e) { set_err(err, errcap, e.what()); return -1; }
}

int zke_fullprove(zke_ctx* x, const uint8_t* inputs, size_t batch, const uint8_t* rs, uint8_t* proofs_out, uint8_t* publics_out,
                  int32_t* status, char* err, size_t errcap) {
    try {
        if (!x || !proofs_out) throw std::runtime_error("null argument");
        require_idle(x);
        zke_ctx::Slot& S = x->slots[0];
        do_witness(x, S, inputs, batch);
        std::string msg;
        int bad = do_prove(x, S, batch, rs, proofs_out, publics_out, status, msg);
        if (bad) { set_err(err, errcap, msg); return bad; }
        return 0;
    } catch (const std::exception& e) { set_err(err, errcap, e.what()); return -1; }
}

int zke_shard_begin(zke_ctx* x, int rank, int world, char* err, size_t errcap) {
    try { if (!x) throw std::runtime_error("null context"); shard_begin(x, rank, world); return 0; }
    catch (const std::exception& e) { set_err(err, errcap, e.what()); return -1; }
}
void* zke_shard_vector(zke_ctx* x, int which, size_t* n_elems) {
    if (!x || !x->zkey || which < 0 || which > 2 || x->lanes_alloc < 1) return nullptr;
    if (n_elems) *n_elems = (size_t)1 << x->zkey->log_n;
    zke_ctx::Lane& L = x->lanes[0];
    return which == 0 ? L.va.p : (which == 1 ? L.vb.p : L.vc.p);
}
int zke_shard_mid(zke_ctx* x, char* err, size_t errcap) {
    try { if (!x) throw std::runtime_error("null context"); shard_mid(x); return 0; }
    catch (const std::exception& e) { set_err(err, errcap, e.what()); return -1; }
}
int zke_shard_end(zke_ctx* x, uint8_t* partial_out, uint8_t* publics_out, char* err, size_t errcap) {
    try { if (!x || !partial_out) throw std::runtime_error("null argument"); shard_end(x, partial_out, publics_out); return 0; }
    catch (const std::exception& e) { set_err(err, errcap, e.what()); return -1; }
}
int zke_shard_combine(const zke_zkey* z, const uint8_t* partials, int world, const uint8_t* rs, uint8_t* proof_out, int32_t* status,
                      char* err, size_t errcap) {
    try {
        if (!z || !partials || !proof_out || world < 1) throw std::runtime_error("bad argument");
        const ShardKeyPoints kp{z->alpha1, z->beta1, z->delta1, z->beta2, z->delta2};
        int bad = shard_combine(&kp, partials, world, rs, proof_out, status);
        if (bad) set_err(err, errcap, "Assert Failed: constraint " + std::to_string(status ? *status : 0));
        return bad;
    } catch (const std::exception& e) { set_err(err, errcap, e.what()); return -1; }
}
int zke_shard_combine_raw(const uint8_t* key_points, const uint8_t* partials, int world, const uint8_t* rs, uint8_t* proof_out,
                          int32_t* status, char* err, size_t errcap) {
    try {
        if (!key_points || !partials || !proof_out || world < 1) throw std::runtime_error("bad argument");
        auto g1 = [&](const uint8_t* q) { return G1AffineH{fq_from_le(q), fq_from_le(q + 32)}; };
        auto g2 = [&](const uint8_t* q) { return G2AffineH{Fq2{fq_from_le(q), fq_from_le(q + 32)}, Fq2{fq_from_le(q + 64), fq_from_le(q + 96)}}; };
        const ShardKeyPoints kp{g1(key_points), g1(key_points + 64), g1(key_points + 128), g2(key_points + 192), g2(key_points + 320)};
        int bad = shard_combine(&kp, partials, world, rs, proof_out, status);
        if (bad) set_err(err, errcap, "Assert Failed: constraint " + std::to_string(status ? *status : 0));
        return bad;
    } catch (const std::exception& e) { set_err(err, errcap, e.what()); return -1; }
}

}

#include "setup.cu"
#include "ptau.cu"
```

### zk-email-verify_b200/csrc/ntt.cu

```cuda
#include "device_engine.cuh"
#include "ntt.cuh"
#include <cstdlib>
#include <type_traits>

namespace zke {
namespace dev {

template <bool SHOUP>
struct Twid {
    Fr w, wq;
    static constexpr uint64_t STRIDE = SHOUP ? 64 : 32;
    __device__ __forceinline__ void load(const uint8_t* base, uint64_t idx) {
        w = Fr::load(base + STRIDE * idx);
        if (SHOUP) wq = Fr::load(base + STRIDE * idx + 32);
    }
    __device__ __forceinline__ Fr mul(const Fr& x) const { return SHOUP ? Fr::mul_shoup(x, w.v, wq.v) : x * w; }
};

static const int MAX_TILE_LOG = 10;

struct Planar {
    uint32_t* sm;
    int tile;
    __device__ __forceinline__ Fr get(int e) const { Fr r; for (int i = 0; i < 8; ++i) r.v[i] = sm[i * tile + e]; return r; }
    __device__ __forceinline__ void put(int e, const Fr& x) const { for (int i = 0; i < 8; ++i) sm[i * tile + e] = x.v[i]; }
};

template <bool DIF, bool SHOUP>
__global__ void __launch_bounds__(1 << (MAX_TILE_LOG - 1))
ntt_pass_kernel(uint8_t* __restrict__ data, const uint8_t* __restrict__ tw, const uint8_t* __restrict__ scale,
                int log_n, int s_lo, int s_hi, int tile_log) {
    extern __shared__ uint32_t smem[];
    const int TILE = 1 << tile_log;
    const int NTT_THREADS = TILE / 2;
    Planar S{smem, TILE};
    const int k = s_hi - s_lo + 1;
    const int J = 1 << k;
    const int L = TILE / J;
    const uint32_t bid = blockIdx.x;
    const bool strided = s_lo > 0;
    uint32_t hi = 0, lo_base = 0;
    if (strided) {
        const uint32_t lo_blocks = (1u << s_lo) / L;
        lo_base = (bid % lo_blocks) * L;
        hi = bid / lo_blocks;
    }
    auto gidx = [&](int j, int l) -> uint32_t {
        return strided ? ((hi << (s_hi + 1)) | ((uint32_t)j << s_lo) | (lo_base + l))
                       : (((bid * L + l) << k) | (uint32_t)j);
    };
    auto sidx = [&](int j, int l) -> int { return strided ? (j * L + l) : (l * J + j); };

    for (int e = threadIdx.x; e < TILE; e += NTT_THREADS) {
        int j, l;
        if (strided) { l = e % L; j = e / L; } else { j = e % J; l = e / J; }
        S.put(e, Fr::load(data + 32ull * gidx(j, l)));
    }
    __syncthreads();

    const int t = threadIdx.x;
    int l, jj;
    if (strided) { l = t % L; jj = t / L; } else { jj = t % (J / 2); l = t / (J / 2); }
    for (int step = 0; step < k; ++step) {
        const int st = DIF ? (s_hi - step) : (s_lo + step);
        const int h = 1 << (st - s_lo);
        const int j0 = ((jj / h) * 2 * h) + (jj % h);
        const int e0 = sidx(j0, l), e1 = sidx(j0 + h, l);
        const uint32_t idx0 = gidx(j0, l);
        const uint32_t tw_i = (idx0 & ((1u << st) - 1)) << (log_n - 1 - st);
        Twid<SHOUP> w;
        w.load(tw, tw_i);
        Fr u = S.get(e0), v = S.get(e1);
        if (DIF) {
            S.put(e0, u + v);
            S.put(e1, w.mul(u - v));
        } else {
            Fr x = w.mul(v);
            S.put(e0, u + x);
            S.put(e1, u - x);
        }
        __syncthreads();
    }
    for (int e = threadIdx.x; e < TILE; e += NTT_THREADS) {
        int j, l2;
        if (strided) { l2 = e % L; j = e / L; } else { j = e % J; l2 = e / J; }
        const uint32_t g = gidx(j, l2);
        Fr x = S.get(e);
        if (scale) { Twid<SHOUP> sc; sc.load(scale, g); x = sc.mul(x); }
        x.store(data + 32ull * g);
    }
}

template <bool DIF, int K, bool STRIDED, bool SHOUP>
__global__ void __launch_bounds__(512, 2)
ntt_pass_fast_kernel(uint8_t* __restrict__ data, const uint8_t* __restrict__ tw, const uint8_t* __restrict__ scale,
                     int log_n, int s_lo_arg) {
    const int s_lo = STRIDED ? s_lo_arg : 0;
    constexpr int TILE_LOG = 10, TILE = 1 << TILE_LOG, J = 1 << K, L_LOG = TILE_LOG - K, L = 1 << L_LOG;
    __shared__ uint4 plane0[TILE], plane1[TILE];
    const int s_hi = s_lo + K - 1;
    const uint32_t bid = blockIdx.x;
    uint32_t hi = 0, lo_base = 0;
    if constexpr (STRIDED) {
        const uint32_t lo_blocks_log = s_lo - L_LOG;
        lo_base = (bid & ((1u << lo_blocks_log) - 1)) << L_LOG;
        hi = bid >> lo_blocks_log;
    }
    auto gidx = [&](uint32_t j, uint32_t l) -> uint32_t {
        return STRIDED ? ((hi << (s_hi + 1)) | (j << s_lo) | (lo_base + l)) : ((((bid << L_LOG) + l) << K) | j);
    };
    auto sidx = [&](uint32_t j, uint32_t l) -> uint32_t { return STRIDED ? ((j << L_LOG) + l) : ((l << K) + j); };
    auto sget = [&](uint32_t e) -> Fr {
        const uint4 a = plane0[e], b = plane1[e];
        Fr r; r.v[0] = a.x; r.v[1] = a.y; r.v[2] = a.z; r.v[3] = a.w; r.v[4] = b.x; r.v[5] = b.y; r.v[6] = b.z; r.v[7] = b.w;
        return r;
    };
    auto sput = [&](uint32_t e, const Fr& x) {
        plane0[e] = make_uint4(x.v[0], x.v[1], x.v[2], x.v[3]);
        plane1[e] = make_uint4(x.v[4], x.v[5], x.v[6], x.v[7]);
    };
#pragma unroll
    for (int r = 0; r < 2; ++r) {
        const uint32_t e = threadIdx.x + r * 512;
        const uint32_t j = STRIDED ? (e >> L_LOG) : (e & (J - 1)), l = STRIDED ? (e & (L - 1)) : (e >> K);
        const uint4* src = reinterpret_cast<const uint4*>(data + 32ull * gidx(j, l));
        plane0[e] = src[0];
        plane1[e] = src[1];
    }
    const uint32_t t = threadIdx.x;
    const uint32_t l = STRIDED ? (t & (L - 1)) : (t >> (K - 1));
    const uint32_t jj = STRIDED ? (t >> L_LOG) : (t & (J / 2 - 1));
    auto stage_of = [&](int step) { return DIF ? (s_hi - step) : (s_lo + step); };
    auto j0_of = [&](int st) -> uint32_t {
        const uint32_t hb = st - s_lo;
        return ((jj >> hb) << (hb + 1)) | (jj & ((1u << hb) - 1));
    };
    auto tw_idx = [&](int st, uint32_t j0) -> uint64_t {
        const uint32_t idx0 = gidx(j0, l);
        return (uint64_t)(idx0 & ((1u << st) - 1)) << (log_n - 1 - st);
    };
    Twid<SHOUP> w_next;
    w_next.load(tw, tw_idx(stage_of(0), j0_of(stage_of(0))));
    __syncthreads();
#pragma unroll
    for (int step = 0; step < K; ++step) {
        const int st = stage_of(step);
        const uint32_t j0 = j0_of(st);
        const uint32_t e0 = sidx(j0, l), e1 = sidx(j0 + (1u << (st - s_lo)), l);
        const Twid<SHOUP> w = w_next;
        if (step + 1 < K) w_next.load(tw, tw_idx(stage_of(step + 1), j0_of(stage_of(step + 1))));
        const Fr u = sget(e0), v = sget(e1);
        const bool trivial = !STRIDED && st == 0;
        if (DIF) {
            sput(e0, u + v);
            sput(e1, trivial ? (u - v) : w.mul(u - v));
        } else {
            const Fr x = trivial ? v : w.mul(v);
            sput(e0, u + x);
            sput(e1, u - x);
        }
        __syncthreads();
    }
#pragma unroll
    for (int r = 0; r < 2; ++r) {
        const uint32_t e = threadIdx.x + r * 512;
        const uint32_t j = STRIDED ? (e >> L_LOG) : (e & (J - 1)), l2 = STRIDED ? (e & (L - 1)) : (e >> K);
        const uint32_t g = gidx(j, l2);
        if (scale) {
            Twid<SHOUP> sc;
            sc.load(scale, g);
            sc.mul(sget(e)).store(data + 32ull * g);
        } else {
            uint4* dst = reinterpret_cast<uint4*>(data + 32ull * g);
            dst[0] = plane0[e];
            dst[1] = plane1[e];
        }
    }
}

template <bool DIF, int K, bool STRIDED, bool SHOUP>
__global__ void __launch_bounds__(128, 3)
ntt_pass_r8_kernel(uint8_t* __restrict__ data, const uint8_t* __restrict__ tw, const uint8_t* __restrict__ scale,
                   int log_n, int s_lo_arg) {
    const int s_lo = STRIDED ? s_lo_arg : 0;
    constexpr int TILE_LOG = 10, TILE = 1 << TILE_LOG, J = 1 << K, L_LOG = TILE_LOG - K, L = 1 << L_LOG;
    constexpr int SM = TILE + TILE / 8;
    __shared__ uint4 plane0[SM], plane1[SM];
    const int s_hi = s_lo + K - 1;
    const uint32_t bid = blockIdx.x;
    uint32_t hi = 0, lo_base = 0;
    if constexpr (STRIDED) {
        const uint32_t lo_blocks_log = s_lo - L_LOG;
        lo_base = (bid & ((1u << lo_blocks_log) - 1)) << L_LOG;
        hi = bid >> lo_blocks_log;
    }
    auto gidx = [&](uint32_t j, uint32_t l) -> uint32_t {
        return STRIDED ? ((hi << (s_hi + 1)) | (j << s_lo) | (lo_base + l)) : ((((bid << L_LOG) + l) << K) | j);
    };
    auto pad = [](uint32_t e) -> uint32_t { return e + (e >> 3); };
    auto sget = [&](uint32_t e) -> Fr {
        const uint4 a = plane0[pad(e)], b = plane1[pad(e)];
        Fr r; r.v[0] = a.x; r.v[1] = a.y; r.v[2] = a.z; r.v[3] = a.w; r.v[4] = b.x; r.v[5] = b.y; r.v[6] = b.z; r.v[7] = b.w;
        return r;
    };
    auto sput = [&](uint32_t e, const Fr& x) {
        plane0[pad(e)] = make_uint4(x.v[0], x.v[1], x.v[2], x.v[3]);
        plane1[pad(e)] = make_uint4(x.v[4], x.v[5], x.v[6], x.v[7]);
    };
#pragma unroll
    for (int r = 0; r < 8; ++r) {
        const uint32_t e = threadIdx.x + r * 128;
        const uint32_t j = STRIDED ? (e >> L_LOG) : (e & (J - 1)), l = STRIDED ? (e & (L - 1)) : (e >> K);
        const uint4* src = reinterpret_cast<const uint4*>(data + 32ull * gidx(j, l));
        plane0[pad(e)] = src[0];
        plane1[pad(e)] = src[1];
    }
    __syncthreads();
    auto round = [&](auto b_tag, auto r_tag) {
        constexpr int B = decltype(b_tag)::value, R = decltype(r_tag)::value, NR = 1 << R;
        constexpr int BP = STRIDED ? B + L_LOG : B;
        constexpr int ITEMS = TILE >> R;
#pragma unroll 1
        for (uint32_t u = threadIdx.x; u < ITEMS; u += 128) {
            const uint32_t base = (u & ((1u << BP) - 1)) | ((u >> BP) << (BP + R));
            const uint32_t j = STRIDED ? (base >> L_LOG) : (base & (J - 1)), l = STRIDED ? (base & (L - 1)) : (base >> K);
            Fr x[NR];
#pragma unroll
            for (int r = 0; r < NR; ++r) x[r] = sget(base + ((uint32_t)r << BP));
#pragma unroll
            for (int qq = 0; qq < R; ++qq) {
                const int q = DIF ? (R - 1 - qq) : qq;
                const int st = s_lo + B + q;
                const bool trivial = !STRIDED && B + q == 0;
                Twid<SHOUP> w[NR / 2];
                if (!trivial) {
#pragma unroll
                    for (int p = 0; p < NR / 2; ++p) {
                        const int r0 = ((p >> q) << (q + 1)) | (p & ((1 << q) - 1));
                        const uint32_t idx0 = gidx(j | ((uint32_t)r0 << B), l);
                        w[p].load(tw, (uint64_t)(idx0 & ((1u << st) - 1)) << (log_n - 1 - st));
                    }
                }
#pragma unroll
                for (int p = 0; p < NR / 2; ++p) {
                    const int r0 = ((p >> q) << (q + 1)) | (p & ((1 << q) - 1)), r1 = r0 | (1 << q);
                    const Fr a = x[r0], b = x[r1];
                    if (DIF) {
                        x[r0] = a + b;
                        x[r1] = trivial ? (a - b) : w[p].mul(a - b);
                    } else {
                        const Fr y = trivial ? b : w[p].mul(b);
                        x[r0] = a + y;
                        x[r1] = a - y;
                    }
                }
            }
#pragma unroll
            for (int r = 0; r < NR; ++r) sput(base + ((uint32_t)r << BP), x[r]);
        }
        __syncthreads();
    };
    using std::integral_constant;
    constexpr int R0 = K >= 3 ? 3 : K, K1 = K - R0, R1 = K1 >= 3 ? 3 : K1, R2 = K1 - R1;
    if (DIF) {
        round(integral_constant<int, K - R0>{}, integral_constant<int, R0>{});
        if constexpr (R1 > 0) round(integral_constant<int, K - R0 - R1>{}, integral_constant<int, R1>{});
        if constexpr (R2 > 0) round(integral_constant<int, 0>{}, integral_constant<int, R2>{});
    } else {
        round(integral_constant<int, 0>{}, integral_constant<int, R0>{});
        if constexpr (R1 > 0) round(integral_constant<int, R0>{}, integral_constant<int, R1>{});
        if constexpr (R2 > 0) round(integral_constant<int, R0 + R1>{}, integral_constant<int, R2>{});
    }
#pragma unroll
    for (int r = 0; r < 8; ++r) {
        const uint32_t e = threadIdx.x + r * 128;
        const uint32_t j = STRIDED ? (e >> L_LOG) : (e & (J - 1)), l2 = STRIDED ? (e & (L - 1)) : (e >> K);
        const uint32_t g = gidx(j, l2);
        if (scale) {
            Twid<SHOUP> sc;
            sc.load(scale, g);
            sc.mul(sget(e)).store(data + 32ull * g);
        } else {
            uint4* dst = reinterpret_cast<uint4*>(data + 32ull * g);
            dst[0] = plane0[pad(e)];
            dst[1] = plane1[pad(e)];
        }
    }
}

template <bool DIF, bool SHOUP>
static bool launch_fast(uint8_t* data, const uint8_t* tw, const uint8_t* scale, int log_n, int s_lo, int s_hi, cudaStream_t st, int log_tw) {
    if (log_n < 10) return false;
    const int k = s_hi - s_lo + 1;
    const uint32_t blocks = 1u << (log_n - 10);
    const bool strided = s_lo > 0;
    if (strided && s_lo < 10 - k) return false;
    static const bool r8 = getenv("ZKE_NTT_R8") && atoi(getenv("ZKE_NTT_R8")) != 0;
#define ZKE_NTT_CASE(KK)                                                                                            \
    case KK:                                                                                                       \
        if (r8) {                                                                                                  \
            if (strided) ntt_pass_r8_kernel<DIF, KK, true, SHOUP><<<blocks, 128, 0, st>>>(data, tw, scale, log_tw, s_lo);  \
            else ntt_pass_r8_kernel<DIF, KK, false, SHOUP><<<blocks, 128, 0, st>>>(data, tw, scale, log_tw, s_lo);         \
        } else if (strided) ntt_pass_fast_kernel<DIF, KK, true, SHOUP><<<blocks, 512, 0, st>>>(data, tw, scale, log_tw, s_lo); \
        else ntt_pass_fast_kernel<DIF, KK, false, SHOUP><<<blocks, 512, 0, st>>>(data, tw, scale, log_tw, s_lo);            \
        return true;
    switch (k) {
        ZKE_NTT_CASE(4) ZKE_NTT_CASE(5) ZKE_NTT_CASE(6) ZKE_NTT_CASE(7) ZKE_NTT_CASE(8)
        default: return false;
    }
#undef ZKE_NTT_CASE
}

static void plan(int log_n, int* lo, int* hi, int* n_pass) {
    int passes = (log_n + 7) / 8;
    int base = log_n / passes, extra = log_n % passes;
    int top = log_n - 1;
    for (int p = 0; p < passes; ++p) {
        int k = base + (p < extra ? 1 : 0);
        hi[p] = top;
        lo[p] = top - k + 1;
        top -= k;
    }
    *n_pass = passes;
}

static void intt_dif_impl(uint8_t* data, const NttTables& T, int log_local, const uint8_t* scale_bitrev, cudaStream_t st) {
    int lo[4], hi[4], np;
    plan(log_local, lo, hi, &np);
    ZKE_COUNT_LAUNCH(np);
    const int tile_log = log_local < MAX_TILE_LOG ? log_local : MAX_TILE_LOG;
    const uint32_t blocks = 1u << (log_local - tile_log);
    for (int p = 0; p < np; ++p) {
        const uint8_t* sc = p == np - 1 ? scale_bitrev : nullptr;
        if (T.shoup ? launch_fast<true, true>(data, T.tw_inv, sc, log_local, lo[p], hi[p], st, T.log_n)
                    : launch_fast<true, false>(data, T.tw_inv, sc, log_local, lo[p], hi[p], st, T.log_n)) continue;
        if (T.shoup) ntt_pass_kernel<true, true><<<blocks, 1 << (tile_log - 1), 32u << tile_log, st>>>(data, T.tw_inv, sc, T.log_n, lo[p], hi[p], tile_log);
        else ntt_pass_kernel<true, false><<<blocks, 1 << (tile_log - 1), 32u << tile_log, st>>>(data, T.tw_inv, sc, T.log_n, lo[p], hi[p], tile_log);
    }
}
static void ntt_dit_impl(uint8_t* data, const NttTables& T, int log_local, cudaStream_t st) {
    int lo[4], hi[4], np;
    plan(log_local, lo, hi, &np);
    ZKE_COUNT_LAUNCH(np);
    const int tile_log = log_local < MAX_TILE_LOG ? log_local : MAX_TILE_LOG;
    const uint32_t blocks = 1u << (log_local - tile_log);
    for (int p = np - 1; p >= 0; --p) {
        if (T.shoup ? launch_fast<false, true>(data, T.tw_fwd, nullptr, log_local, lo[p], hi[p], st, T.log_n)
                    : launch_fast<false, false>(data, T.tw_fwd, nullptr, log_local, lo[p], hi[p], st, T.log_n)) continue;
        if (T.shoup) ntt_pass_kernel<false, true><<<blocks, 1 << (tile_log - 1), 32u << tile_log, st>>>(data, T.tw_fwd, nullptr, T.log_n, lo[p], hi[p], tile_log);
        else ntt_pass_kernel<false, false><<<blocks, 1 << (tile_log - 1), 32u << tile_log, st>>>(data, T.tw_fwd, nullptr, T.log_n, lo[p], hi[p], tile_log);
    }
}
void launch_intt_dif(uint8_t* data, const NttTables& T, const uint8_t* scale_bitrev, cudaStream_t st) { intt_dif_impl(data, T, T.log_n, scale_bitrev, st); }
void launch_ntt_dit(uint8_t* data, const NttTables& T, cudaStream_t st) { ntt_dit_impl(data, T, T.log_n, st); }
void launch_intt_dif_block(uint8_t* block, const NttTables& T, int log_local, const uint8_t* scale_block, cudaStream_t st) { intt_dif_impl(block, T, log_local, scale_block, st); }
void launch_ntt_dit_block(uint8_t* block, const NttTables& T, int log_local, cudaStream_t st) { ntt_dit_impl(block, T, log_local, st); }

template <bool DIF, int LOGG, bool SHOUP>
__global__ void __launch_bounds__(128)
ntt_cross_kernel(uint8_t* __restrict__ data, const uint8_t* __restrict__ tw, int log_n, uint32_t col0, uint32_t n_cols) {
    constexpr int G = 1 << LOGG;
    const uint32_t t = blockIdx.x * blockDim.x + threadIdx.x;
    if (t >= n_cols) return;
    const int log_m = log_n - LOGG;
    const uint32_t j = col0 + t;
    Fr x[G];
#pragma unroll
    for (int g = 0; g < G; ++g) x[g] = Fr::load(data + 32ull * (((uint32_t)g << log_m) + j));
#pragma unroll
    for (int step = 0; step < LOGG; ++step) {
        const int sb = DIF ? (LOGG - 1 - step) : step;
        const int st = log_m + sb;
#pragma unroll
        for (int g0 = 0; g0 < G; ++g0) {
            if (g0 & (1 << sb)) continue;
            const int g1 = g0 | (1 << sb);
            const uint32_t idx0 = ((uint32_t)g0 << log_m) + j;
            const uint64_t tw_i = (uint64_t)(idx0 & ((1u << st) - 1)) << (log_n - 1 - st);
            Twid<SHOUP> w;
            w.load(tw, tw_i);
            const Fr u = x[g0], v = x[g1];
            if (DIF) {
                x[g0] = u + v;
                x[g1] = w.mul(u - v);
            } else {
                const Fr y = w.mul(v);
                x[g0] = u + y;
                x[g1] = u - y;
            }
        }
    }
#pragma unroll
    for (int g = 0; g < G; ++g) x[g].store(data + 32ull * (((uint32_t)g << log_m) + j));
}
template <bool DIF, bool SHOUP>
static void launch_cross(uint8_t* data, const uint8_t* tw, int log_n, int log_g, uint32_t col0, uint32_t n_cols, cudaStream_t st) {
    const uint32_t blocks = (n_cols + 127) / 128;
    switch (log_g) {
        case 1: ntt_cross_kernel<DIF, 1, SHOUP><<<blocks, 128, 0, st>>>(data, tw, log_n, col0, n_cols); break;
        case 2: ntt_cross_kernel<DIF, 2, SHOUP><<<blocks, 128, 0, st>>>(data, tw, log_n, col0, n_cols); break;
        case 3: ntt_cross_kernel<DIF, 3, SHOUP><<<blocks, 128, 0, st>>>(data, tw, log_n, col0, n_cols); break;
        default: break;
    }
    ZKE_COUNT_LAUNCH(1);
}
void launch_intt_cross(uint8_t* data, const NttTables& T, int log_g, uint32_t col0, uint32_t n_cols, cudaStream_t st) {
    if (T.shoup) launch_cross<true, true>(data, T.tw_inv, T.log_n, log_g, col0, n_cols, st);
    else launch_cross<true, false>(data, T.tw_inv, T.log_n, log_g, col0, n_cols, st);
}
void launch_ntt_cross(uint8_t* data, const NttTables& T, int log_g, uint32_t col0, uint32_t n_cols, cudaStream_t st) {
    if (T.shoup) launch_cross<false, true>(data, T.tw_fwd, T.log_n, log_g, col0, n_cols, st);
    else launch_cross<false, false>(data, T.tw_fwd, T.log_n, log_g, col0, n_cols, st);
}

__global__ void hadamard_kernel(const uint8_t* __restrict__ a, const uint8_t* __restrict__ b, uint8_t* __restrict__ c, uint32_t n) {
    uint32_t i = blockIdx.x * blockDim.x + threadIdx.x;
    if (i >= n) return;
    (Fr::load(a + 32ull * i) * Fr::load(b + 32ull * i)).store(c + 32ull * i);
}
void launch_hadamard(const uint8_t* a, const uint8_t* b, uint8_t* c, uint32_t n, cudaStream_t st) {
    hadamard_kernel<<<(n + 255) / 256, 256, 0, st>>>(a, b, c, n);
    ZKE_COUNT_LAUNCH(1);
}

__global__ void quotient_kernel(const uint8_t* __restrict__ a, const uint8_t* __restrict__ b, const uint8_t* __restrict__ c,
                                uint8_t* __restrict__ d, uint32_t n) {
    uint32_t i = blockIdx.x * blockDim.x + threadIdx.x;
    if (i >= n) return;
    Fr x = Fr::load(a + 32ull * i) * Fr::load(b + 32ull * i) - Fr::load(c + 32ull * i);
    x.from_mont().store(d + 32ull * i);
}
void launch_quotient(const uint8_t* a, const uint8_t* b, const uint8_t* c, uint8_t* d, uint32_t n, cudaStream_t st) {
    quotient_kernel<<<(n + 255) / 256, 256, 0, st>>>(a, b, c, d, n);
    ZKE_COUNT_LAUNCH(1);
}
__global__ void quotient_cols_kernel(const uint8_t* __restrict__ a, const uint8_t* __restrict__ b, const uint8_t* __restrict__ c,
                                     uint8_t* __restrict__ d, uint32_t n_threads, int log_m, int log_cols, uint32_t col0) {
    const uint32_t t = blockIdx.x * blockDim.x + threadIdx.x;
    if (t >= n_threads) return;
    const uint32_t i = ((t >> log_cols) << log_m) + col0 + (t & ((1u << log_cols) - 1));
    Fr x = Fr::load(a + 32ull * i) * Fr::load(b + 32ull * i) - Fr::load(c + 32ull * i);
    x.from_mont().store(d + 32ull * i);
}
void launch_quotient_cols(const uint8_t* a, const uint8_t* b, const uint8_t* c, uint8_t* d, int log_n, int log_g, uint32_t col0, uint32_t n_cols_log, cudaStream_t st) {
    const uint32_t n_threads = (1u << log_g) << n_cols_log;
    quotient_cols_kernel<<<(n_threads + 255) / 256, 256, 0, st>>>(a, b, c, d, n_threads, log_n - log_g, (int)n_cols_log, col0);
    ZKE_COUNT_LAUNCH(1);
}

}
}
```

### zk-email-verify_b200/csrc/ntt.cuh

```cuda
#pragma once
#include <cstdint>
#include <cuda_runtime.h>

namespace zke {
namespace dev {

struct NttTables {
    const uint8_t* tw_fwd;
    const uint8_t* tw_inv;
    int log_n;
    bool shoup;
};

void launch_intt_dif(uint8_t* data, const NttTables& T, const uint8_t* scale_bitrev, cudaStream_t st);
void launch_ntt_dit(uint8_t* data, const NttTables& T, cudaStream_t st);
void launch_intt_dif_block(uint8_t* block, const NttTables& T, int log_local, const uint8_t* scale_block, cudaStream_t st);
void launch_ntt_dit_block(uint8_t* block, const NttTables& T, int log_local, cudaStream_t st);
void launch_intt_cross(uint8_t* data, const NttTables& T, int log_g, uint32_t col0, uint32_t n_cols, cudaStream_t st);
void launch_ntt_cross(uint8_t* data, const NttTables& T, int log_g, uint32_t col0, uint32_t n_cols, cudaStream_t st);
void launch_quotient_cols(const uint8_t* a, const uint8_t* b, const uint8_t* c, uint8_t* d, int log_n, int log_g, uint32_t col0, uint32_t n_cols_log, cudaStream_t st);
void launch_hadamard(const uint8_t* a, const uint8_t* b, uint8_t* c, uint32_t n, cudaStream_t st);
void launch_quotient(const uint8_t* a, const uint8_t* b, const uint8_t* c, uint8_t* d, uint32_t n, cudaStream_t st);

}
}
```

Before: 47.82.

## Fuse iNTT/NTT round trip and quotient into pass kernels, drop Shoup path

Replaces the separate inverse-DIF, forward-DIT and quotient launches with a round-trip routine. The last inverse pass applies the coset scale, and the final forward pass on the C vector computes a*b-c and writes the quotient directly, which removes the standalone quotient kernel and one full read/write of the vectors. It also removes the optional Shoup twiddle path and the radix-8 kernel, and refactors the fast pass into a reusable FastTile struct. Removing the radix-8 variant may lose a faster specialised path, and the fused quotient in the final pass adds extra global loads inside that kernel.

```diff
diff --git a/zk-email-verify_b200/csrc/engine.cu b/zk-email-verify_b200/csrc/engine.cu
--- a/zk-email-verify_b200/csrc/engine.cu
+++ b/zk-email-verify_b200/csrc/engine.cu
@@ -560,51 +560,13 @@
     R.coef_r = x->coef_r.p; R.n_vars = x->n_vars;
 }
 
-namespace {
-struct ShoupPair { U256 w, wq; };
-U256 mul_lo256(const U256& a, const U256& b) {
-    uint64_t t[4] = {0, 0, 0, 0};
-    for (int i = 0; i < 4; ++i) {
-        u128 c = 0;
-        for (int j = 0; i + j < 4; ++j) {
-            c += (u128)a.v[j] * b.v[i] + t[i + j];
-            t[i + j] = (uint64_t)c;
-            c >>= 64;
-        }
-    }
-    return U256{{t[0], t[1], t[2], t[3]}};
-}
-const U256& fr_neg_inv256() {
-    static const U256 v = [] {
-        const U256& p = fr_params().p;
-        U256 y = {{(uint64_t)0 - fr_params().inv, 0, 0, 0}};
-        for (int it = 0; it < 2; ++it) {
-            U256 t = mul_lo256(p, y), two = {{2, 0, 0, 0}}, d;
-            u256_sub(d, two, t);
-            y = mul_lo256(y, d);
-        }
-        U256 zero = {{0, 0, 0, 0}}, n;
-        u256_sub(n, zero, y);
-        return n;
-    }();
-    return v;
-}
-ShoupPair shoup_pair(const Fr& w) { return ShoupPair{w.to_u256(), mul_lo256(w.m, fr_neg_inv256())}; }
-}
-
 static void build_ntt_tables(zke_ctx* x, unsigned log_n) {
     const size_t N = (size_t)1 << log_n;
     const Fr omega = fr_root_of_unity(log_n), omega_inv = omega.inv();
     const Fr g = fr_root_of_unity(log_n + 1);
     const Fr n_inv = Fr::from_u64(N).inv();
-    bool shoup = false;
-    if (const char* e = getenv("ZKE_NTT_SHOUP")) shoup = atoi(e) != 0;
-    const size_t esz = shoup ? 64 : 32;
-    std::vector<uint8_t> fw(esz * std::max<size_t>(1, N / 2)), iv(esz * std::max<size_t>(1, N / 2)), cs(esz * N);
-    auto put = [&](std::vector<uint8_t>& tab, size_t i, const Fr& w) {
-        if (shoup) { const ShoupPair sp = shoup_pair(w); memcpy(&tab[64 * i], sp.w.v, 32); memcpy(&tab[64 * i + 32], sp.wq.v, 32); }
-        else memcpy(&tab[32 * i], w.m.v, 32);
-    };
+    std::vector<uint8_t> fw(32 * std::max<size_t>(1, N / 2)), iv(32 * std::max<size_t>(1, N / 2)), cs(32 * N);
+    auto put = [&](std::vector<uint8_t>& tab, size_t i, const Fr& w) { memcpy(&tab[32 * i], w.m.v, 32); };
     const unsigned T = std::max(1u, std::min(16u, std::thread::hardware_concurrency()));
     std::vector<std::thread> th;
     for (unsigned t = 0; t < T; ++t) {
@@ -631,7 +593,7 @@
     for (auto& t : th) t.join();
     if (N == 1) { put(fw, 0, Fr::one()); put(iv, 0, Fr::one()); }
     x->tw_fwd.upload(fw); x->tw_inv.upload(iv); x->coset_scale.upload(cs);
-    x->ntt.tw_fwd = x->tw_fwd.p; x->ntt.tw_inv = x->tw_inv.p; x->ntt.log_n = (int)log_n; x->ntt.shoup = shoup;
+    x->ntt.tw_fwd = x->tw_fwd.p; x->ntt.tw_inv = x->tw_inv.p; x->ntt.log_n = (int)log_n;
 }
 
 static void open_lanes(zke_ctx* x, size_t N, int prio_least, int prio_greatest) {
@@ -829,13 +791,9 @@
         dev::launch_build_ab(x->r1cs, w, L.va.p, L.vb.p, L.vc.p, N, flag, st);
         if (prof) { t1 = x->mark(st); x->spans.push_back({ZKE_STAGE_MATVEC, t0, t1}); t0 = t1; }
         if (hv != st) { CUDA_OK(cudaEventRecord(L.ev[0], st)); CUDA_OK(cudaStreamWaitEvent(hv, L.ev[0], 0)); }
-        dev::launch_intt_dif(L.va.p, x->ntt, x->coset_scale.p, hv);
-        dev::launch_intt_dif(L.vb.p, x->ntt, x->coset_scale.p, hv);
-        dev::launch_intt_dif(L.vc.p, x->ntt, x->coset_scale.p, hv);
-        dev::launch_ntt_dit(L.va.p, x->ntt, hv);
-        dev::launch_ntt_dit(L.vb.p, x->ntt, hv);
-        dev::launch_ntt_dit(L.vc.p, x->ntt, hv);
-        dev::launch_quotient(L.va.p, L.vb.p, L.vc.p, L.vd.p, N, hv);
+        dev::launch_ntt_roundtrip(L.va.p, x->ntt, x->coset_scale.p, nullptr, nullptr, nullptr, hv);
+        dev::launch_ntt_roundtrip(L.vb.p, x->ntt, x->coset_scale.p, nullptr, nullptr, nullptr, hv);
+        dev::launch_ntt_roundtrip(L.vc.p, x->ntt, x->coset_scale.p, L.va.p, L.vb.p, L.vd.p, hv);
         CHECK_LAUNCH();
         if (hv != st) CUDA_OK(cudaEventRecord(L.ev[1], hv));
         if (prof) { t1 = x->mark(st); x->spans.push_back({ZKE_STAGE_NTT, t0, t1}); t0 = t1; }
@@ -1033,8 +991,7 @@
     cudaStream_t st = L.st;
     const size_t block_off = ((size_t)x->shard_rank << log_m);
     for (uint8_t* v : {L.va.p, L.vb.p, L.vc.p}) {
-        dev::launch_intt_dif_block(v + 32 * block_off, x->ntt, log_m, x->coset_scale.p + (x->ntt.shoup ? 64 : 32) * block_off, st);
-        dev::launch_ntt_dit_block(v + 32 * block_off, x->ntt, log_m, st);
+        dev::launch_ntt_roundtrip_block(v + 32 * block_off, x->ntt, log_m, x->coset_scale.p + 32 * block_off, st);
     }
     CHECK_LAUNCH();
     CUDA_OK(cudaStreamSynchronize(st));
diff --git a/zk-email-verify_b200/csrc/ntt.cu b/zk-email-verify_b200/csrc/ntt.cu
--- a/zk-email-verify_b200/csrc/ntt.cu
+++ b/zk-email-verify_b200/csrc/ntt.cu
@@ -1,21 +1,9 @@
 #include "device_engine.cuh"
 #include "ntt.cuh"
 #include <cstdlib>
-#include <type_traits>
 
 namespace zke {
 namespace dev {
-
-template <bool SHOUP>
-struct Twid {
-    Fr w, wq;
-    static constexpr uint64_t STRIDE = SHOUP ? 64 : 32;
-    __device__ __forceinline__ void load(const uint8_t* base, uint64_t idx) {
-        w = Fr::load(base + STRIDE * idx);
-        if (SHOUP) wq = Fr::load(base + STRIDE * idx + 32);
-    }
-    __device__ __forceinline__ Fr mul(const Fr& x) const { return SHOUP ? Fr::mul_shoup(x, w.v, wq.v) : x * w; }
-};
 
 static const int MAX_TILE_LOG = 10;
 
@@ -26,9 +14,14 @@
     __device__ __forceinline__ void put(int e, const Fr& x) const { for (int i = 0; i < 8; ++i) sm[i * tile + e] = x.v[i]; }
 };
 
-template <bool DIF, bool SHOUP>
+__device__ __forceinline__ void store_quotient(const uint8_t* qa, const uint8_t* qb, uint8_t* qd, uint32_t g, const Fr& x) {
+    (Fr::load(qa + 32ull * g) * Fr::load(qb + 32ull * g) - x).from_mont().store(qd + 32ull * g);
+}
+
+template <bool DIF>
 __global__ void __launch_bounds__(1 << (MAX_TILE_LOG - 1))
 ntt_pass_kernel(uint8_t* __restrict__ data, const uint8_t* __restrict__ tw, const uint8_t* __restrict__ scale,
+                const uint8_t* qa, const uint8_t* qb, uint8_t* qd,
                 int log_n, int s_lo, int s_hi, int tile_log) {
     extern __shared__ uint32_t smem[];
     const int TILE = 1 << tile_log;
@@ -68,14 +61,13 @@
         const int e0 = sidx(j0, l), e1 = sidx(j0 + h, l);
         const uint32_t idx0 = gidx(j0, l);
         const uint32_t tw_i = (idx0 & ((1u << st) - 1)) << (log_n - 1 - st);
-        Twid<SHOUP> w;
-        w.load(tw, tw_i);
+        const Fr w = Fr::load(tw + 32ull * tw_i);
         Fr u = S.get(e0), v = S.get(e1);
         if (DIF) {
             S.put(e0, u + v);
-            S.put(e1, w.mul(u - v));
+            S.put(e1, (u - v) * w);
         } else {
-            Fr x = w.mul(v);
+            Fr x = v * w;
             S.put(e0, u + x);
             S.put(e1, u - x);
         }
@@ -86,230 +78,151 @@
         if (strided) { l2 = e % L; j = e / L; } else { j = e % J; l2 = e / J; }
         const uint32_t g = gidx(j, l2);
         Fr x = S.get(e);
-        if (scale) { Twid<SHOUP> sc; sc.load(scale, g); x = sc.mul(x); }
-        x.store(data + 32ull * g);
-    }
-}
-
-template <bool DIF, int K, bool STRIDED, bool SHOUP>
-__global__ void __launch_bounds__(512, 2)
-ntt_pass_fast_kernel(uint8_t* __restrict__ data, const uint8_t* __restrict__ tw, const uint8_t* __restrict__ scale,
-                     int log_n, int s_lo_arg) {
-    const int s_lo = STRIDED ? s_lo_arg : 0;
-    constexpr int TILE_LOG = 10, TILE = 1 << TILE_LOG, J = 1 << K, L_LOG = TILE_LOG - K, L = 1 << L_LOG;
-    __shared__ uint4 plane0[TILE], plane1[TILE];
-    const int s_hi = s_lo + K - 1;
-    const uint32_t bid = blockIdx.x;
-    uint32_t hi = 0, lo_base = 0;
-    if constexpr (STRIDED) {
-        const uint32_t lo_blocks_log = s_lo - L_LOG;
-        lo_base = (bid & ((1u << lo_blocks_log) - 1)) << L_LOG;
-        hi = bid >> lo_blocks_log;
-    }
-    auto gidx = [&](uint32_t j, uint32_t l) -> uint32_t {
-        return STRIDED ? ((hi << (s_hi + 1)) | (j << s_lo) | (lo_base + l)) : ((((bid << L_LOG) + l) << K) | j);
-    };
-    auto sidx = [&](uint32_t j, uint32_t l) -> uint32_t { return STRIDED ? ((j << L_LOG) + l) : ((l << K) + j); };
-    auto sget = [&](uint32_t e) -> Fr {
+        if (scale) x = x * Fr::load(scale + 32ull * g);
+        if (qd) store_quotient(qa, qb, qd, g, x);
+        else x.store(data + 32ull * g);
+    }
+}
+
+template <int K, bool STRIDED>
+struct FastTile {
+    static constexpr int TILE_LOG = 10, TILE = 1 << TILE_LOG, J = 1 << K, L_LOG = TILE_LOG - K, L = 1 << L_LOG;
+    uint4* plane0;
+    uint4* plane1;
+    int s_lo, s_hi, log_n;
+    uint32_t bid, hi, lo_base, l, jj;
+
+    __device__ __forceinline__ FastTile(uint4* p0, uint4* p1, int s_lo_arg, int log_n_) : plane0(p0), plane1(p1), log_n(log_n_) {
+        s_lo = STRIDED ? s_lo_arg : 0;
+        s_hi = s_lo + K - 1;
+        bid = blockIdx.x;
+        hi = 0; lo_base = 0;
+        if constexpr (STRIDED) {
+            const uint32_t lo_blocks_log = s_lo - L_LOG;
+            lo_base = (bid & ((1u << lo_blocks_log) - 1)) << L_LOG;
+            hi = bid >> lo_blocks_log;
+        }
+        const uint32_t t = threadIdx.x;
+        l = STRIDED ? (t & (L - 1)) : (t >> (K - 1));
+        jj = STRIDED ? (t >> L_LOG) : (t & (J / 2 - 1));
+    }
+    __device__ __forceinline__ uint32_t gidx(uint32_t j, uint32_t l2) const {
+        return STRIDED ? ((hi << (s_hi + 1)) | (j << s_lo) | (lo_base + l2)) : ((((bid << L_LOG) + l2) << K) | j);
+    }
+    __device__ __forceinline__ uint32_t sidx(uint32_t j, uint32_t l2) const { return STRIDED ? ((j << L_LOG) + l2) : ((l2 << K) + j); }
+    __device__ __forceinline__ void jl(uint32_t e, uint32_t& j, uint32_t& l2) const {
+        j = STRIDED ? (e >> L_LOG) : (e & (J - 1));
+        l2 = STRIDED ? (e & (L - 1)) : (e >> K);
+    }
+    __device__ __forceinline__ Fr get(uint32_t e) const {
         const uint4 a = plane0[e], b = plane1[e];
         Fr r; r.v[0] = a.x; r.v[1] = a.y; r.v[2] = a.z; r.v[3] = a.w; r.v[4] = b.x; r.v[5] = b.y; r.v[6] = b.z; r.v[7] = b.w;
         return r;
-    };
-    auto sput = [&](uint32_t e, const Fr& x) {
+    }
+    __device__ __forceinline__ void put(uint32_t e, const Fr& x) const {
         plane0[e] = make_uint4(x.v[0], x.v[1], x.v[2], x.v[3]);
         plane1[e] = make_uint4(x.v[4], x.v[5], x.v[6], x.v[7]);
-    };
-#pragma unroll
-    for (int r = 0; r < 2; ++r) {
-        const uint32_t e = threadIdx.x + r * 512;
-        const uint32_t j = STRIDED ? (e >> L_LOG) : (e & (J - 1)), l = STRIDED ? (e & (L - 1)) : (e >> K);
-        const uint4* src = reinterpret_cast<const uint4*>(data + 32ull * gidx(j, l));
-        plane0[e] = src[0];
-        plane1[e] = src[1];
-    }
-    const uint32_t t = threadIdx.x;
-    const uint32_t l = STRIDED ? (t & (L - 1)) : (t >> (K - 1));
-    const uint32_t jj = STRIDED ? (t >> L_LOG) : (t & (J / 2 - 1));
-    auto stage_of = [&](int step) { return DIF ? (s_hi - step) : (s_lo + step); };
-    auto j0_of = [&](int st) -> uint32_t {
+    }
+    __device__ __forceinline__ void load(const uint8_t* data) const {
+#pragma unroll
+        for (int r = 0; r < 2; ++r) {
+            const uint32_t e = threadIdx.x + r * 512;
+            uint32_t j, l2;
+            jl(e, j, l2);
+            const uint4* src = reinterpret_cast<const uint4*>(data + 32ull * gidx(j, l2));
+            plane0[e] = src[0];
+            plane1[e] = src[1];
+        }
+    }
+    __device__ __forceinline__ uint32_t j0_of(int st) const {
         const uint32_t hb = st - s_lo;
         return ((jj >> hb) << (hb + 1)) | (jj & ((1u << hb) - 1));
-    };
-    auto tw_idx = [&](int st, uint32_t j0) -> uint64_t {
-        const uint32_t idx0 = gidx(j0, l);
-        return (uint64_t)(idx0 & ((1u << st) - 1)) << (log_n - 1 - st);
-    };
-    Twid<SHOUP> w_next;
-    w_next.load(tw, tw_idx(stage_of(0), j0_of(stage_of(0))));
+    }
+    __device__ __forceinline__ Fr twiddle(const uint8_t* tw, int st) const {
+        const uint32_t idx0 = gidx(j0_of(st), l);
+        return Fr::load(tw + 32ull * ((uint64_t)(idx0 & ((1u << st) - 1)) << (log_n - 1 - st)));
+    }
+    template <bool DIF, int N_STAGES>
+    __device__ __forceinline__ void stages(const uint8_t* tw, int st_first, bool skip0) const {
+        if constexpr (N_STAGES > 0) {
+            Fr w_next = twiddle(tw, st_first);
+#pragma unroll
+            for (int step = 0; step < N_STAGES; ++step) {
+                const int st = DIF ? st_first - step : st_first + step;
+                const uint32_t j0 = j0_of(st);
+                const uint32_t e0 = sidx(j0, l), e1 = sidx(j0 + (1u << (st - s_lo)), l);
+                const Fr w = w_next;
+                if (step + 1 < N_STAGES) w_next = twiddle(tw, DIF ? st - 1 : st + 1);
+                const Fr u = get(e0), v = get(e1);
+                const bool trivial = skip0 && st == 0;
+                if (DIF) {
+                    put(e0, u + v);
+                    put(e1, trivial ? (u - v) : (u - v) * w);
+                } else {
+                    const Fr x = trivial ? v : v * w;
+                    put(e0, u + x);
+                    put(e1, u - x);
+                }
+                __syncthreads();
+            }
+        }
+    }
+    __device__ __forceinline__ void store(uint8_t* data, const uint8_t* scale, const uint8_t* qa, const uint8_t* qb, uint8_t* qd) const {
+#pragma unroll
+        for (int r = 0; r < 2; ++r) {
+            const uint32_t e = threadIdx.x + r * 512;
+            uint32_t j, l2;
+            jl(e, j, l2);
+            const uint32_t g = gidx(j, l2);
+            if (scale) {
+                (get(e) * Fr::load(scale + 32ull * g)).store(data + 32ull * g);
+            } else if (qd) {
+                store_quotient(qa, qb, qd, g, get(e));
+            } else {
+                uint4* dst = reinterpret_cast<uint4*>(data + 32ull * g);
+                dst[0] = plane0[e];
+                dst[1] = plane1[e];
+            }
+        }
+    }
+};
+
+template <bool DIF, int K, bool STRIDED>
+__global__ void __launch_bounds__(512, 2)
+ntt_pass_fast_kernel(uint8_t* __restrict__ data, const uint8_t* __restrict__ tw, const uint8_t* __restrict__ scale,
+                     const uint8_t* qa, const uint8_t* qb, uint8_t* qd, int log_n, int s_lo_arg) {
+    __shared__ uint4 plane0[1 << 10], plane1[1 << 10];
+    const FastTile<K, STRIDED> T(plane0, plane1, s_lo_arg, log_n);
+    T.load(data);
     __syncthreads();
-#pragma unroll
-    for (int step = 0; step < K; ++step) {
-        const int st = stage_of(step);
-        const uint32_t j0 = j0_of(st);
-        const uint32_t e0 = sidx(j0, l), e1 = sidx(j0 + (1u << (st - s_lo)), l);
-        const Twid<SHOUP> w = w_next;
-        if (step + 1 < K) w_next.load(tw, tw_idx(stage_of(step + 1), j0_of(stage_of(step + 1))));
-        const Fr u = sget(e0), v = sget(e1);
-        const bool trivial = !STRIDED && st == 0;
-        if (DIF) {
-            sput(e0, u + v);
-            sput(e1, trivial ? (u - v) : w.mul(u - v));
-        } else {
-            const Fr x = trivial ? v : w.mul(v);
-            sput(e0, u + x);
-            sput(e1, u - x);
-        }
-        __syncthreads();
-    }
-#pragma unroll
-    for (int r = 0; r < 2; ++r) {
-        const uint32_t e = threadIdx.x + r * 512;
-        const uint32_t j = STRIDED ? (e >> L_LOG) : (e & (J - 1)), l2 = STRIDED ? (e & (L - 1)) : (e >> K);
-        const uint32_t g = gidx(j, l2);
-        if (scale) {
-            Twid<SHOUP> sc;
-            sc.load(scale, g);
-            sc.mul(sget(e)).store(data + 32ull * g);
-        } else {
-            uint4* dst = reinterpret_cast<uint4*>(data + 32ull * g);
-            dst[0] = plane0[e];
-            dst[1] = plane1[e];
-        }
-    }
-}
-
-template <bool DIF, int K, bool STRIDED, bool SHOUP>
-__global__ void __launch_bounds__(128, 3)
-ntt_pass_r8_kernel(uint8_t* __restrict__ data, const uint8_t* __restrict__ tw, const uint8_t* __restrict__ scale,
-                   int log_n, int s_lo_arg) {
-    const int s_lo = STRIDED ? s_lo_arg : 0;
-    constexpr int TILE_LOG = 10, TILE = 1 << TILE_LOG, J = 1 << K, L_LOG = TILE_LOG - K, L = 1 << L_LOG;
-    constexpr int SM = TILE + TILE / 8;
-    __shared__ uint4 plane0[SM], plane1[SM];
-    const int s_hi = s_lo + K - 1;
-    const uint32_t bid = blockIdx.x;
-    uint32_t hi = 0, lo_base = 0;
-    if constexpr (STRIDED) {
-        const uint32_t lo_blocks_log = s_lo - L_LOG;
-        lo_base = (bid & ((1u << lo_blocks_log) - 1)) << L_LOG;
-        hi = bid >> lo_blocks_log;
-    }
-    auto gidx = [&](uint32_t j, uint32_t l) -> uint32_t {
-        return STRIDED ? ((hi << (s_hi + 1)) | (j << s_lo) | (lo_base + l)) : ((((bid << L_LOG) + l) << K) | j);
-    };
-    auto pad = [](uint32_t e) -> uint32_t { return e + (e >> 3); };
-    auto sget = [&](uint32_t e) -> Fr {
-        const uint4 a = plane0[pad(e)], b = plane1[pad(e)];
-        Fr r; r.v[0] = a.x; r.v[1] = a.y; r.v[2] = a.z; r.v[3] = a.w; r.v[4] = b.x; r.v[5] = b.y; r.v[6] = b.z; r.v[7] = b.w;
-        return r;
-    };
-    auto sput = [&](uint32_t e, const Fr& x) {
-        plane0[pad(e)] = make_uint4(x.v[0], x.v[1], x.v[2], x.v[3]);
-        plane1[pad(e)] = make_uint4(x.v[4], x.v[5], x.v[6], x.v[7]);
-    };
-#pragma unroll
-    for (int r = 0; r < 8; ++r) {
-        const uint32_t e = threadIdx.x + r * 128;
-        const uint32_t j = STRIDED ? (e >> L_LOG) : (e & (J - 1)), l = STRIDED ? (e & (L - 1)) : (e >> K);
-        const uint4* src = reinterpret_cast<const uint4*>(data + 32ull * gidx(j, l));
-        plane0[pad(e)] = src[0];
-        plane1[pad(e)] = src[1];
-    }
-    __syncthreads();
-    auto round = [&](auto b_tag, auto r_tag) {
-        constexpr int B = decltype(b_tag)::value, R = decltype(r_tag)::value, NR = 1 << R;
-        constexpr int BP = STRIDED ? B + L_LOG : B;
-        constexpr int ITEMS = TILE >> R;
-#pragma unroll 1
-        for (uint32_t u = threadIdx.x; u < ITEMS; u += 128) {
-            const uint32_t base = (u & ((1u << BP) - 1)) | ((u >> BP) << (BP + R));
-            const uint32_t j = STRIDED ? (base >> L_LOG) : (base & (J - 1)), l = STRIDED ? (base & (L - 1)) : (base >> K);
-            Fr x[NR];
-#pragma unroll
-            for (int r = 0; r < NR; ++r) x[r] = sget(base + ((uint32_t)r << BP));
-#pragma unroll
-            for (int qq = 0; qq < R; ++qq) {
-                const int q = DIF ? (R - 1 - qq) : qq;
-                const int st = s_lo + B + q;
-                const bool trivial = !STRIDED && B + q == 0;
-                Twid<SHOUP> w[NR / 2];
-                if (!trivial) {
-#pragma unroll
-                    for (int p = 0; p < NR / 2; ++p) {
-                        const int r0 = ((p >> q) << (q + 1)) | (p & ((1 << q) - 1));
-                        const uint32_t idx0 = gidx(j | ((uint32_t)r0 << B), l);
-                        w[p].load(tw, (uint64_t)(idx0 & ((1u << st) - 1)) << (log_n - 1 - st));
-                    }
-                }
-#pragma unroll
-                for (int p = 0; p < NR / 2; ++p) {
-                    const int r0 = ((p >> q) << (q + 1)) | (p & ((1 << q) - 1)), r1 = r0 | (1 << q);
-                    const Fr a = x[r0], b = x[r1];
-                    if (DIF) {
-                        x[r0] = a + b;
-                        x[r1] = trivial ? (a - b) : w[p].mul(a - b);
-                    } else {
-                        const Fr y = trivial ? b : w[p].mul(b);
-                        x[r0] = a + y;
-                        x[r1] = a - y;
-                    }
-                }
-            }
-#pragma unroll
-            for (int r = 0; r < NR; ++r) sput(base + ((uint32_t)r << BP), x[r]);
-        }
-        __syncthreads();
-    };
-    using std::integral_constant;
-    constexpr int R0 = K >= 3 ? 3 : K, K1 = K - R0, R1 = K1 >= 3 ? 3 : K1, R2 = K1 - R1;
-    if (DIF) {
-        round(integral_constant<int, K - R0>{}, integral_constant<int, R0>{});
-        if constexpr (R1 > 0) round(integral_constant<int, K - R0 - R1>{}, integral_constant<int, R1>{});
-        if constexpr (R2 > 0) round(integral_constant<int, 0>{}, integral_constant<int, R2>{});
-    } else {
-        round(integral_constant<int, 0>{}, integral_constant<int, R0>{});
-        if constexpr (R1 > 0) round(integral_constant<int, R0>{}, integral_constant<int, R1>{});
-        if constexpr (R2 > 0) round(integral_constant<int, R0 + R1>{}, integral_constant<int, R2>{});
-    }
-#pragma unroll
-    for (int r = 0; r < 8; ++r) {
-        const uint32_t e = threadIdx.x + r * 128;
-        const uint32_t j = STRIDED ? (e >> L_LOG) : (e & (J - 1)), l2 = STRIDED ? (e & (L - 1)) : (e >> K);
-        const uint32_t g = gidx(j, l2);
-        if (scale) {
-            Twid<SHOUP> sc;
-            sc.load(scale, g);
-            sc.mul(sget(e)).store(data + 32ull * g);
-        } else {
-            uint4* dst = reinterpret_cast<uint4*>(data + 32ull * g);
-            dst[0] = plane0[pad(e)];
-            dst[1] = plane1[pad(e)];
-        }
-    }
-}
-
-template <bool DIF, bool SHOUP>
-static bool launch_fast(uint8_t* data, const uint8_t* tw, const uint8_t* scale, int log_n, int s_lo, int s_hi, cudaStream_t st, int log_tw) {
+    T.template stages<DIF, K>(tw, DIF ? T.s_hi : T.s_lo, true);
+    T.store(data, scale, qa, qb, qd);
+}
+
+#define ZKE_NTT_SWITCH_K(k, CASE)                                                                                   \
+    switch (k) {                                                                                                   \
+        CASE(4) CASE(5) CASE(6) CASE(7) CASE(8)                                                                    \
+        default: return false;                                                                                     \
+    }
+
+template <bool DIF>
+static bool launch_fast(uint8_t* data, const uint8_t* tw, const uint8_t* scale, const uint8_t* qa, const uint8_t* qb, uint8_t* qd,
+                        int log_n, int s_lo, int s_hi, cudaStream_t st, int log_tw) {
     if (log_n < 10) return false;
     const int k = s_hi - s_lo + 1;
     const uint32_t blocks = 1u << (log_n - 10);
     const bool strided = s_lo > 0;
     if (strided && s_lo < 10 - k) return false;
-    static const bool r8 = getenv("ZKE_NTT_R8") && atoi(getenv("ZKE_NTT_R8")) != 0;
 #define ZKE_NTT_CASE(KK)                                                                                            \
     case KK:                                                                                                       \
-        if (r8) {                                                                                                  \
-            if (strided) ntt_pass_r8_kernel<DIF, KK, true, SHOUP><<<blocks, 128, 0, st>>>(data, tw, scale, log_tw, s_lo);  \
-            else ntt_pass_r8_kernel<DIF, KK, false, SHOUP><<<blocks, 128, 0, st>>>(data, tw, scale, log_tw, s_lo);         \
-        } else if (strided) ntt_pass_fast_kernel<DIF, KK, true, SHOUP><<<blocks, 512, 0, st>>>(data, tw, scale, log_tw, s_lo); \
-        else ntt_pass_fast_kernel<DIF, KK, false, SHOUP><<<blocks, 512, 0, st>>>(data, tw, scale, log_tw, s_lo);            \
+        if (strided) ntt_pass_fast_kernel<DIF, KK, true><<<blocks, 512, 0, st>>>(data, tw, scale, qa, qb, qd, log_tw, s_lo); \
+        else ntt_pass_fast_kernel<DIF, KK, false><<<blocks, 512, 0, st>>>(data, tw, scale, qa, qb, qd, log_tw, s_lo);        \
         return true;
-    switch (k) {
-        ZKE_NTT_CASE(4) ZKE_NTT_CASE(5) ZKE_NTT_CASE(6) ZKE_NTT_CASE(7) ZKE_NTT_CASE(8)
-        default: return false;
-    }
+    ZKE_NTT_SWITCH_K(k, ZKE_NTT_CASE)
 #undef ZKE_NTT_CASE
 }
+
+#undef ZKE_NTT_SWITCH_K
 
 static void plan(int log_n, int* lo, int* hi, int* n_pass) {
     int passes = (log_n + 7) / 8;
@@ -324,39 +237,39 @@
     *n_pass = passes;
 }
 
-static void intt_dif_impl(uint8_t* data, const NttTables& T, int log_local, const uint8_t* scale_bitrev, cudaStream_t st) {
+static void roundtrip_impl(uint8_t* data, const NttTables& T, int log_local, const uint8_t* scale,
+                           const uint8_t* qa, const uint8_t* qb, uint8_t* qd, cudaStream_t st) {
     int lo[4], hi[4], np;
     plan(log_local, lo, hi, &np);
-    ZKE_COUNT_LAUNCH(np);
+    const int last = np - 1;
+    if (log_local >= MAX_TILE_LOG) {
+        bool ok = true;
+        for (int p = 0; p < np; ++p)
+            ok = ok && launch_fast<true>(data, T.tw_inv, p == last ? scale : nullptr, nullptr, nullptr, nullptr, log_local, lo[p], hi[p], st, T.log_n);
+        for (int p = last; p >= 0; --p)
+            ok = ok && launch_fast<false>(data, T.tw_fwd, nullptr, qa, qb, p == 0 ? qd : nullptr, log_local, lo[p], hi[p], st, T.log_n);
+        if (!ok) throw std::runtime_error("NTT pass schedule without a tiled kernel");
+        ZKE_COUNT_LAUNCH(2 * np);
+        return;
+    }
     const int tile_log = log_local < MAX_TILE_LOG ? log_local : MAX_TILE_LOG;
     const uint32_t blocks = 1u << (log_local - tile_log);
-    for (int p = 0; p < np; ++p) {
-        const uint8_t* sc = p == np - 1 ? scale_bitrev : nullptr;
-        if (T.shoup ? launch_fast<true, true>(data, T.tw_inv, sc, log_local, lo[p], hi[p], st, T.log_n)
-                    : launch_fast<true, false>(data, T.tw_inv, sc, log_local, lo[p], hi[p], st, T.log_n)) continue;
-        if (T.shoup) ntt_pass_kernel<true, true><<<blocks, 1 << (tile_log - 1), 32u << tile_log, st>>>(data, T.tw_inv, sc, T.log_n, lo[p], hi[p], tile_log);
-        else ntt_pass_kernel<true, false><<<blocks, 1 << (tile_log - 1), 32u << tile_log, st>>>(data, T.tw_inv, sc, T.log_n, lo[p], hi[p], tile_log);
-    }
-}
-static void ntt_dit_impl(uint8_t* data, const NttTables& T, int log_local, cudaStream_t st) {
-    int lo[4], hi[4], np;
-    plan(log_local, lo, hi, &np);
-    ZKE_COUNT_LAUNCH(np);
-    const int tile_log = log_local < MAX_TILE_LOG ? log_local : MAX_TILE_LOG;
-    const uint32_t blocks = 1u << (log_local - tile_log);
-    for (int p = np - 1; p >= 0; --p) {
-        if (T.shoup ? launch_fast<false, true>(data, T.tw_fwd, nullptr, log_local, lo[p], hi[p], st, T.log_n)
-                    : launch_fast<false, false>(data, T.tw_fwd, nullptr, log_local, lo[p], hi[p], st, T.log_n)) continue;
-        if (T.shoup) ntt_pass_kernel<false, true><<<blocks, 1 << (tile_log - 1), 32u << tile_log, st>>>(data, T.tw_fwd, nullptr, T.log_n, lo[p], hi[p], tile_log);
-        else ntt_pass_kernel<false, false><<<blocks, 1 << (tile_log - 1), 32u << tile_log, st>>>(data, T.tw_fwd, nullptr, T.log_n, lo[p], hi[p], tile_log);
-    }
-}
-void launch_intt_dif(uint8_t* data, const NttTables& T, const uint8_t* scale_bitrev, cudaStream_t st) { intt_dif_impl(data, T, T.log_n, scale_bitrev, st); }
-void launch_ntt_dit(uint8_t* data, const NttTables& T, cudaStream_t st) { ntt_dit_impl(data, T, T.log_n, st); }
-void launch_intt_dif_block(uint8_t* block, const NttTables& T, int log_local, const uint8_t* scale_block, cudaStream_t st) { intt_dif_impl(block, T, log_local, scale_block, st); }
-void launch_ntt_dit_block(uint8_t* block, const NttTables& T, int log_local, cudaStream_t st) { ntt_dit_impl(block, T, log_local, st); }
-
-template <bool DIF, int LOGG, bool SHOUP>
+    const unsigned threads = 1u << (tile_log > 0 ? tile_log - 1 : 0), smem = 32u << tile_log;
+    for (int p = 0; p < np; ++p)
+        ntt_pass_kernel<true><<<blocks, threads, smem, st>>>(data, T.tw_inv, p == last ? scale : nullptr, nullptr, nullptr, nullptr, T.log_n, lo[p], hi[p], tile_log);
+    for (int p = last; p >= 0; --p)
+        ntt_pass_kernel<false><<<blocks, threads, smem, st>>>(data, T.tw_fwd, nullptr, qa, qb, p == 0 ? qd : nullptr, T.log_n, lo[p], hi[p], tile_log);
+    ZKE_COUNT_LAUNCH(2 * np);
+}
+
+void launch_ntt_roundtrip(uint8_t* data, const NttTables& T, const uint8_t* scale_bitrev, const uint8_t* qa, const uint8_t* qb, uint8_t* qd, cudaStream_t st) {
+    roundtrip_impl(data, T, T.log_n, scale_bitrev, qa, qb, qd, st);
+}
+void launch_ntt_roundtrip_block(uint8_t* block, const NttTables& T, int log_local, const uint8_t* scale_block, cudaStream_t st) {
+    roundtrip_impl(block, T, log_local, scale_block, nullptr, nullptr, nullptr, st);
+}
+
+template <bool DIF, int LOGG>
 __global__ void __launch_bounds__(128)
 ntt_cross_kernel(uint8_t* __restrict__ data, const uint8_t* __restrict__ tw, int log_n, uint32_t col0, uint32_t n_cols) {
     constexpr int G = 1 << LOGG;
@@ -377,14 +290,13 @@
             const int g1 = g0 | (1 << sb);
             const uint32_t idx0 = ((uint32_t)g0 << log_m) + j;
             const uint64_t tw_i = (uint64_t)(idx0 & ((1u << st) - 1)) << (log_n - 1 - st);
-            Twid<SHOUP> w;
-            w.load(tw, tw_i);
+            const Fr w = Fr::load(tw + 32ull * tw_i);
             const Fr u = x[g0], v = x[g1];
             if (DIF) {
                 x[g0] = u + v;
-                x[g1] = w.mul(u - v);
+                x[g1] = (u - v) * w;
             } else {
-                const Fr y = w.mul(v);
+                const Fr y = v * w;
                 x[g0] = u + y;
                 x[g1] = u - y;
             }
@@ -393,24 +305,22 @@
 #pragma unroll
     for (int g = 0; g < G; ++g) x[g].store(data + 32ull * (((uint32_t)g << log_m) + j));
 }
-template <bool DIF, bool SHOUP>
+template <bool DIF>
 static void launch_cross(uint8_t* data, const uint8_t* tw, int log_n, int log_g, uint32_t col0, uint32_t n_cols, cudaStream_t st) {
     const uint32_t blocks = (n_cols + 127) / 128;
     switch (log_g) {
-        case 1: ntt_cross_kernel<DIF, 1, SHOUP><<<blocks, 128, 0, st>>>(data, tw, log_n, col0, n_cols); break;
-        case 2: ntt_cross_kernel<DIF, 2, SHOUP><<<blocks, 128, 0, st>>>(data, tw, log_n, col0, n_cols); break;
-        case 3: ntt_cross_kernel<DIF, 3, SHOUP><<<blocks, 128, 0, st>>>(data, tw, log_n, col0, n_cols); break;
+        case 1: ntt_cross_kernel<DIF, 1><<<blocks, 128, 0, st>>>(data, tw, log_n, col0, n_cols); break;
+        case 2: ntt_cross_kernel<DIF, 2><<<blocks, 128, 0, st>>>(data, tw, log_n, col0, n_cols); break;
+        case 3: ntt_cross_kernel<DIF, 3><<<blocks, 128, 0, st>>>(data, tw, log_n, col0, n_cols); break;
         default: break;
     }
     ZKE_COUNT_LAUNCH(1);
 }
 void launch_intt_cross(uint8_t* data, const NttTables& T, int log_g, uint32_t col0, uint32_t n_cols, cudaStream_t st) {
-    if (T.shoup) launch_cross<true, true>(data, T.tw_inv, T.log_n, log_g, col0, n_cols, st);
-    else launch_cross<true, false>(data, T.tw_inv, T.log_n, log_g, col0, n_cols, st);
+    launch_cross<true>(data, T.tw_inv, T.log_n, log_g, col0, n_cols, st);
 }
 void launch_ntt_cross(uint8_t* data, const NttTables& T, int log_g, uint32_t col0, uint32_t n_cols, cudaStream_t st) {
-    if (T.shoup) launch_cross<false, true>(data, T.tw_fwd, T.log_n, log_g, col0, n_cols, st);
-    else launch_cross<false, false>(data, T.tw_fwd, T.log_n, log_g, col0, n_cols, st);
+    launch_cross<false>(data, T.tw_fwd, T.log_n, log_g, col0, n_cols, st);
 }
 
 __global__ void hadamard_kernel(const uint8_t* __restrict__ a, const uint8_t* __restrict__ b, uint8_t* __restrict__ c, uint32_t n) {
@@ -423,17 +333,6 @@
     ZKE_COUNT_LAUNCH(1);
 }
 
-__global__ void quotient_kernel(const uint8_t* __restrict__ a, const uint8_t* __restrict__ b, const uint8_t* __restrict__ c,
-                                uint8_t* __restrict__ d, uint32_t n) {
-    uint32_t i = blockIdx.x * blockDim.x + threadIdx.x;
-    if (i >= n) return;
-    Fr x = Fr::load(a + 32ull * i) * Fr::load(b + 32ull * i) - Fr::load(c + 32ull * i);
-    x.from_mont().store(d + 32ull * i);
-}
-void launch_quotient(const uint8_t* a, const uint8_t* b, const uint8_t* c, uint8_t* d, uint32_t n, cudaStream_t st) {
-    quotient_kernel<<<(n + 255) / 256, 256, 0, st>>>(a, b, c, d, n);
-    ZKE_COUNT_LAUNCH(1);
-}
 __global__ void quotient_cols_kernel(const uint8_t* __restrict__ a, const uint8_t* __restrict__ b, const uint8_t* __restrict__ c,
                                      uint8_t* __restrict__ d, uint32_t n_threads, int log_m, int log_cols, uint32_t col0) {
     const uint32_t t = blockIdx.x * blockDim.x + threadIdx.x;
diff --git a/zk-email-verify_b200/csrc/ntt.cuh b/zk-email-verify_b200/csrc/ntt.cuh
--- a/zk-email-verify_b200/csrc/ntt.cuh
+++ b/zk-email-verify_b200/csrc/ntt.cuh
@@ -9,18 +9,14 @@
     const uint8_t* tw_fwd;
     const uint8_t* tw_inv;
     int log_n;
-    bool shoup;
 };
 
-void launch_intt_dif(uint8_t* data, const NttTables& T, const uint8_t* scale_bitrev, cudaStream_t st);
-void launch_ntt_dit(uint8_t* data, const NttTables& T, cudaStream_t st);
-void launch_intt_dif_block(uint8_t* block, const NttTables& T, int log_local, const uint8_t* scale_block, cudaStream_t st);
-void launch_ntt_dit_block(uint8_t* block, const NttTables& T, int log_local, cudaStream_t st);
+void launch_ntt_roundtrip(uint8_t* data, const NttTables& T, const uint8_t* scale_bitrev, const uint8_t* qa, const uint8_t* qb, uint8_t* qd, cudaStream_t st);
+void launch_ntt_roundtrip_block(uint8_t* block, const NttTables& T, int log_local, const uint8_t* scale_block, cudaStream_t st);
 void launch_intt_cross(uint8_t* data, const NttTables& T, int log_g, uint32_t col0, uint32_t n_cols, cudaStream_t st);
 void launch_ntt_cross(uint8_t* data, const NttTables& T, int log_g, uint32_t col0, uint32_t n_cols, cudaStream_t st);
 void launch_quotient_cols(const uint8_t* a, const uint8_t* b, const uint8_t* c, uint8_t* d, int log_n, int log_g, uint32_t col0, uint32_t n_cols_log, cudaStream_t st);
 void launch_hadamard(const uint8_t* a, const uint8_t* b, uint8_t* c, uint32_t n, cudaStream_t st);
-void launch_quotient(const uint8_t* a, const uint8_t* b, const uint8_t* c, uint8_t* d, uint32_t n, cudaStream_t st);
 
 }
 }
```

Result: slower. 46.97 (median of 6 runs) (-1.8%).
